# saiakarsh193/GenVox

Measured on AMD Instinct MI355X. Metric: mel-frames/sec (teacher-forced batch), higher is better.
Workload: dtype f32

## Files before the change

genvox_amd/csrc/gemm_f32.hip:

```cpp
#include "gvx_kernels.h"

#include <cstdlib>

namespace gvx {

using f32x16 = __attribute__((ext_vector_type(16))) float;

constexpr int BK32 = 32;

__device__ __forceinline__ long row_off(const RowMap& m, int row) {
    return (long)(row / m.R) * m.s1 + (long)(row % m.R) * m.s0;
}

template <int WR, int WC, int TM, int TN, bool KMAJ = false, int BK = BK32>
__device__ __forceinline__ void gemm_f32_body(const GemmParams& p, const int block_x, const int tid, float* smem) {
    constexpr int LDS_LD = BK + 4;
    static_assert(BK == 32 || (BK == 64 && !KMAJ), "k-tiles of 32, or 64 for the row-major form");
    constexpr int BM = WR * TM * 32;
    constexpr int BN = WC * TN * 32;
    constexpr int NT = WR * WC * 64;
    constexpr int TPR = BK / 4;
    constexpr int RPP = NT / TPR;
    constexpr int A_V4 = (BM + RPP - 1) / RPP;
    constexpr int B_V4 = (BN + RPP - 1) / RPP;
    static_assert(!KMAJ || NT == 256, "the K-major loaders are written for 256 threads");
    float* As = smem;
    float* Bs = smem + 2 * BM * LDS_LD;

    const int lane = tid & 63, wave = tid >> 6;
    const int wr = wave / WC, wc = wave % WC;
    const int r = lane & 31, h = lane >> 5;
    const int n_tiles = (p.N + BN - 1) / BN;
    const int mt = block_x / n_tiles, nt = block_x % n_tiles;
    const int m0 = p.m_begin + mt * BM, n0 = nt * BN;
    const int k_begin = p.splitk > 1 ? (int)blockIdx.y * p.kchunk : 0;
    const int k_end = p.splitk > 1 ? min(p.K, k_begin + p.kchunk) : p.K;
    const long slice = p.splitk > 1 ? 0 : (long)blockIdx.y;
    const float* const Ab = p.A + slice * p.a_slice;
    const float* const Wb = p.W + slice * p.w_slice;
    float* const Cout = p.C + (p.splitk > 1 ? (long)blockIdx.y * p.c_split : slice * p.c_slice);

    const int ld_row = tid / TPR, ld_c4 = tid % TPR;
    const float* a_ptr[A_V4]; bool a_ok[A_V4];
    const float* b_ptr[B_V4]; bool b_ok[B_V4];
    constexpr int A_MQ = BM / 4, B_NQ = BN / 4;
    constexpr int A_P = (8 * A_MQ + 255) / 256, B_P = (8 * B_NQ + 255) / 256;
    const int amq = tid % A_MQ, akq = tid / A_MQ, bnq = tid % B_NQ, bkq = tid / B_NQ;
    const int a_col = min(m0 + 4 * amq, p.M - 4), b_col = min(n0 + 4 * bnq, p.N - 4);
    int ak_g[A_P], ak_i[A_P], bk_g[B_P], bk_i[B_P];
    long a_safe = 0, b_safe = 0;
    float4 ka_reg[A_P][4], kb_reg[B_P][4];
    if (KMAJ) {
#pragma unroll
        for (int i = 0; i < A_P; ++i) { const int k = k_begin + 4 * (akq + (256 / A_MQ) * i); ak_g[i] = k / p.amap.R; ak_i[i] = k - ak_g[i] * p.amap.R; }
#pragma unroll
        for (int i = 0; i < B_P; ++i) { const int k = k_begin + 4 * (bkq + (256 / B_NQ) * i); bk_g[i] = k / p.wmap.R; bk_i[i] = k - bk_g[i] * p.wmap.R; }
        a_safe = row_off(p.amap, k_begin); b_safe = row_off(p.wmap, k_begin);
    }
    if (!KMAJ) {
#pragma unroll
        for (int i = 0; i < A_V4; ++i) {
            int m = m0 + ld_row + RPP * i;
            a_ok[i] = m < p.M;
            a_ptr[i] = Ab + (a_ok[i] ? row_off(p.amap, m) : 0);
        }
#pragma unroll
        for (int i = 0; i < B_V4; ++i) {
            int n = n0 + ld_row + RPP * i;
            b_ok[i] = n < p.N;
            b_ptr[i] = Wb + (b_ok[i] ? (long)n * p.ldw : 0);
        }
    }
    float4 a_reg[A_V4], b_reg[B_V4];

#define GEMM_KMAJ_LOAD(NP, QPP, KQ, KG, KI, MAP, SAFE, PTR, COL, REG)                                        \
        _Pragma("unroll") for (int i = 0; i < NP; ++i) {                                                    \
            const int c_ = KQ + QPP * i;                                                                    \
            if (c_ < BK / 4) {                                                                              \
                const int kq_ = (K0_) + 4 * c_;                                                             \
                int g_ = KG[i], x_ = KI[i];                                                                 \
                _Pragma("unroll") for (int j = 0; j < 4; ++j) {                                             \
                    const bool ok_ = kq_ + j < k_end;                                                       \
                    REG[i][j] = *reinterpret_cast<const float4*>(PTR + (ok_ ? (long)g_ * MAP.s1 + (long)x_ * MAP.s0 : SAFE) + COL); \
                    if (++x_ == MAP.R) { x_ = 0; ++g_; }                                                    \
                }                                                                                           \
                x_ = KI[i] + BK; g_ = KG[i];                                                                \
                while (x_ >= MAP.R) { x_ -= MAP.R; ++g_; }                                                  \
                KI[i] = x_; KG[i] = g_;                                                                     \
            }                                                                                               \
        }
#define GEMM_LOAD_TILE(K0)                                                                                  \
    if (KMAJ) {                                                                                             \
        const int K0_ = (K0);                                                                               \
        GEMM_KMAJ_LOAD(A_P, (256 / A_MQ), akq, ak_g, ak_i, p.amap, a_safe, Ab, a_col, ka_reg)              \
        GEMM_KMAJ_LOAD(B_P, (256 / B_NQ), bkq, bk_g, bk_i, p.wmap, b_safe, Wb, b_col, kb_reg)              \
    } else                                                                                                  \
    {                                                                                                       \
        const int k_ = (K0) + 4 * ld_c4;                                                                    \
        const bool k_ok_ = k_ < k_end;                                                                      \
        const long a_koff_ = (long)(k_ >> 3) * p.a_kblk + (k_ & 7);                                         \
        _Pragma("unroll") for (int i = 0; i < A_V4; ++i) {                                                  \
            if (BM % RPP != 0 && ld_row + RPP * i >= BM) continue;                                          \
            a_reg[i] = *reinterpret_cast<const float4*>(a_ptr[i] + (k_ok_ ? a_koff_ : 0));                  \
        }                                                                                                   \
        _Pragma("unroll") for (int i = 0; i < B_V4; ++i) {                                                  \
            if (BN % RPP != 0 && ld_row + RPP * i >= BN) continue;                                          \
            b_reg[i] = *reinterpret_cast<const float4*>(b_ptr[i] + (k_ok_ ? k_ : 0));                       \
        }                                                                                                   \
    }
#define GEMM_KMAJ_STORE(NP, QPP, KQ, SM, ROWS, RQ, REG, BUF)                                                 \
        _Pragma("unroll") for (int i = 0; i < NP; ++i) {                                                    \
            const int c_ = KQ + QPP * i;                                                                    \
            if (c_ < BK / 4) {                                                                              \
                float* d_ = &SM[((BUF) * ROWS + 4 * RQ) * LDS_LD + 4 * c_];                                 \
                const int kq_ = (KS_) + 4 * c_;    \
                const bool o0_ = kq_ < k_end, o1_ = kq_ + 1 < k_end, o2_ = kq_ + 2 < k_end, o3_ = kq_ + 3 < k_end;   \
                *reinterpret_cast<float4*>(d_) = make_float4(o0_ ? REG[i][0].x : 0.f, o1_ ? REG[i][1].x : 0.f, o2_ ? REG[i][2].x : 0.f, o3_ ? REG[i][3].x : 0.f);              \
                *reinterpret_cast<float4*>(d_ + LDS_LD) = make_float4(o0_ ? REG[i][0].y : 0.f, o1_ ? REG[i][1].y : 0.f, o2_ ? REG[i][2].y : 0.f, o3_ ? REG[i][3].y : 0.f);     \
                *reinterpret_cast<float4*>(d_ + 2 * LDS_LD) = make_float4(o0_ ? REG[i][0].z : 0.f, o1_ ? REG[i][1].z : 0.f, o2_ ? REG[i][2].z : 0.f, o3_ ? REG[i][3].z : 0.f); \
                *reinterpret_cast<float4*>(d_ + 3 * LDS_LD) = make_float4(o0_ ? REG[i][0].w : 0.f, o1_ ? REG[i][1].w : 0.f, o2_ ? REG[i][2].w : 0.f, o3_ ? REG[i][3].w : 0.f); \
            }                                                                                               \
        }
#define GEMM_STORE_TILE(BUF, K0)                                                                            \
    if (KMAJ) {                                                                                             \
        const int KS_ = (K0);                                                                               \
        GEMM_KMAJ_STORE(A_P, (256 / A_MQ), akq, As, BM, amq, ka_reg, BUF)                                   \
        GEMM_KMAJ_STORE(B_P, (256 / B_NQ), bkq, Bs, BN, bnq, kb_reg, BUF)                                   \
    } else                                                                                                  \
    {                                                                                                       \
        const bool s_ok_ = (K0) + 4 * ld_c4 < k_end;    \
        _Pragma("unroll") for (int i = 0; i < A_V4; ++i)                                                    \
            if (BM % RPP == 0 || ld_row + RPP * i < BM)                                                     \
                *reinterpret_cast<float4*>(&As[((BUF) * BM + ld_row + RPP * i) * LDS_LD + 4 * ld_c4]) =     \
                    make_float4(s_ok_ ? a_reg[i].x : 0.f, s_ok_ ? a_reg[i].y : 0.f, s_ok_ ? a_reg[i].z : 0.f, s_ok_ ? a_reg[i].w : 0.f); \
        _Pragma("unroll") for (int i = 0; i < B_V4; ++i)                                                    \
            if (BN % RPP == 0 || ld_row + RPP * i < BN)                                                     \
                *reinterpret_cast<float4*>(&Bs[((BUF) * BN + ld_row + RPP * i) * LDS_LD + 4 * ld_c4]) =     \
                    make_float4(s_ok_ ? b_reg[i].x : 0.f, s_ok_ ? b_reg[i].y : 0.f, s_ok_ ? b_reg[i].z : 0.f, s_ok_ ? b_reg[i].w : 0.f); \
    }
#define GEMM_COMPUTE_TILE(BUF) GEMM_COMPUTE_KGS(BUF, 0, BK / 8)
#define GEMM_COMPUTE_KGS(BUF, KG0, KG1)              \
    {                                                                                                       \
        const float* a_base = &As[((BUF) * BM + wr * TM * 32 + r) * LDS_LD + 4 * h];                        \
        const float* b_base = &Bs[((BUF) * BN + wc * TN * 32 + r) * LDS_LD + 4 * h];                        \
        _Pragma("unroll") for (int kg = (KG0); kg < (KG1); ++kg) {                                          \
            float4 af[TM], bf[TN];                                                                          \
            _Pragma("unroll") for (int i = 0; i < TM; ++i)                                                  \
                af[i] = *reinterpret_cast<const float4*>(a_base + i * 32 * LDS_LD + 8 * kg);                \
            _Pragma("unroll") for (int j = 0; j < TN; ++j)                                                  \
                bf[j] = *reinterpret_cast<const float4*>(b_base + j * 32 * LDS_LD + 8 * kg);                \
            _Pragma("unroll") for (int i = 0; i < TM; ++i)                                                  \
                _Pragma("unroll") for (int j = 0; j < TN; ++j) {                                            \
                    acc[i][j] = __builtin_amdgcn_mfma_f32_32x32x2f32(af[i].x, bf[j].x, acc[i][j], 0, 0, 0); \
                    acc[i][j] = __builtin_amdgcn_mfma_f32_32x32x2f32(af[i].y, bf[j].y, acc[i][j], 0, 0, 0); \
                    acc[i][j] = __builtin_amdgcn_mfma_f32_32x32x2f32(af[i].z, bf[j].z, acc[i][j], 0, 0, 0); \
                    acc[i][j] = __builtin_amdgcn_mfma_f32_32x32x2f32(af[i].w, bf[j].w, acc[i][j], 0, 0, 0); \
                }                                                                                           \
        }                                                                                                   \
    }

    f32x16 acc[TM][TN];
#pragma unroll
    for (int i = 0; i < TM; ++i)
#pragma unroll
        for (int j = 0; j < TN; ++j)
#pragma unroll
            for (int q = 0; q < 16; ++q) acc[i][j][q] = 0.f;

    const int nkt = (k_end - k_begin + BK - 1) / BK;
    GEMM_LOAD_TILE(k_begin)
    GEMM_STORE_TILE(0, k_begin)
    __syncthreads();
    int kt = 0;
    for (; kt + 1 < nkt; ++kt) {
        const int cur = kt & 1;
        GEMM_LOAD_TILE(k_begin + (kt + 1) * BK)
        __builtin_amdgcn_sched_barrier(0);
        GEMM_COMPUTE_KGS(cur, 0, BK / 8 - 1)
        __builtin_amdgcn_sched_barrier(0);
        GEMM_COMPUTE_KGS(cur, BK / 8 - 1, BK / 8)
        GEMM_STORE_TILE(cur ^ 1, k_begin + (kt + 1) * BK)
        __syncthreads();
    }
    GEMM_COMPUTE_TILE(kt & 1)
#undef GEMM_LOAD_TILE
#undef GEMM_KMAJ_LOAD
#undef GEMM_KMAJ_STORE
#undef GEMM_STORE_TILE
#undef GEMM_COMPUTE_TILE
#undef GEMM_COMPUTE_KGS

#pragma unroll
    for (int i = 0; i < TM; ++i) {
#pragma unroll
        for (int q = 0; q < 16; ++q) {
            const int m = m0 + (wr * TM + i) * 32 + (q & 3) + 8 * (q >> 2) + 4 * h;
            if (m >= p.M) continue;
            const long c_off = row_off(p.cmap, m);
            const int grp = m / p.cmap.R, idx = m - grp * p.cmap.R;
            const bool live = !p.row_len || idx < p.row_len[grp];
            const bool halo_front = p.c_halo > 0 && idx < p.c_halo;
            const bool halo_back = p.c_halo > 0 && idx >= p.cmap.R - p.c_halo;
            const long halo_step = (long)p.c_halo * p.cmap.s0;
#pragma unroll
            for (int j = 0; j < TN; ++j) {
                const int n = n0 + (wc * TN + j) * 32 + r;
                if (n >= p.N) continue;
                float v = acc[i][j][q];
                if (p.bias) v += p.bias[n];
                if (p.act == ACT_RELU) v = fmaxf(v, 0.f);
                else if (p.act == ACT_TANH) v = tanhf(v);
                if (p.keep) v = p.keep[(long)m * p.keep_ld + n] ? 2.f * v : 0.f;
                const long col = (long)(n >> 3) * p.c_nblk + (n & 7);
                Cout[c_off + col] = live ? v : 0.f;
                if (halo_front) Cout[c_off - halo_step + col] = 0.f;
                if (halo_back) Cout[c_off + halo_step + col] = 0.f;
            }
        }
    }
}

template <int WR, int WC, int TM, int TN, bool KMAJ = false, int BK = BK32>
__global__ __launch_bounds__(WR * WC * 64) void gemm_f32_kernel(GemmParams p) {
    extern __shared__ __attribute__((aligned(16))) float smem[];
    gemm_f32_body<WR, WC, TM, TN, KMAJ, BK>(p, (int)blockIdx.x, (int)threadIdx.x, smem);
}

template <int WR, int WC, int TM, int TN, int BK = BK32>
static size_t lds_bytes_cfg() { return (size_t)2 * (WR * TM * 32 + WC * TN * 32) * (BK + 4) * sizeof(float); }

template <int WR, int WC, int TM, int TN, bool KMAJ = false, int BK = BK32>
static hipError_t init_cfg() {
    return hipFuncSetAttribute(reinterpret_cast<const void*>(gemm_f32_kernel<WR, WC, TM, TN, KMAJ, BK>),
                               hipFuncAttributeMaxDynamicSharedMemorySize, (int)lds_bytes_cfg<WR, WC, TM, TN, BK>());
}

hipError_t gemm_init() {
    hipError_t e = init_cfg<2, 2, 2, 2>();
    if (e != hipSuccess) return e;
    e = init_cfg<2, 2, 1, 2>();
    if (e != hipSuccess) return e;
    e = init_cfg<4, 1, 1, 3>();
    if (e != hipSuccess) return e;
    e = init_cfg<2, 3, 1, 1>();
    if (e != hipSuccess) return e;
    e = init_cfg<4, 2, 1, 2>();
    if (e != hipSuccess) return e;
    e = init_cfg<2, 2, 1, 1>();
    if (e != hipSuccess) return e;
    e = init_cfg<2, 2, 2, 2, true>();
    if (e != hipSuccess) return e;
    e = init_cfg<2, 2, 1, 2, true>();
    if (e != hipSuccess) return e;
    return init_cfg<4, 1, 1, 1>();
}

template <int WR, int WC, int TM, int TN, bool KMAJ = false, int BK = BK32>
static hipError_t launch_cfg(const GemmParams& p, hipStream_t s) {
    constexpr int BM = WR * TM * 32, BN = WC * TN * 32;
    const int grid = ((p.M - p.m_begin + BM - 1) / BM) * ((p.N + BN - 1) / BN);
    gemm_f32_kernel<WR, WC, TM, TN, KMAJ, BK><<<dim3(grid, p.splitk > 1 ? p.splitk : p.slices > 1 ? p.slices : 1), dim3(WR * WC * 64), lds_bytes_cfg<WR, WC, TM, TN, BK>(), s>>>(p);
    return hipGetLastError();
}

static bool four_waves() {
    static const bool on = [] { const char* e = std::getenv("GVX_GEMM_8W"); return e && e[0] == '0'; }();
    return on;
}

GemmPlan plan_gemm(const GemmParams& p) {
    GemmPlan pl{hipSuccess, 0, 0};
    if (p.M <= 0 || p.N <= 0) return pl;
    if (p.slices > 1 && (p.splitk > 1 || p.kmajor || p.keep || p.slices > 65535)) { pl.err = hipErrorInvalidValue; return pl; }
    if (p.kmajor) {
        if ((p.M & 3) || (p.N & 3) || p.M < 4 || p.N < 4 || ((p.amap.s0 | p.amap.s1 | p.wmap.s0 | p.wmap.s1) & 3)) { pl.err = hipErrorInvalidValue; return pl; }
        const long t128 = (long)((p.M + 127) / 128) * ((p.N + 127) / 128);
        pl.tile = t128 < 384 ? 2212 : 2222;
        return pl;
    }
    if (p.K & 3) { pl.err = hipErrorInvalidValue; return pl; }
    if (p.N <= 32) { pl.tile = 4111; return pl; }
    if (p.N <= 96) {
        pl.tile = p.M - p.m_begin <= 4096 ? 2311 : 4113;
        return pl;
    }
    const long n_tiles = (long)((p.N + 127) / 128) * (p.slices > 1 ? p.slices : 1), tiles128 = (long)((p.M + 127) / 128) * n_tiles;
    if (tiles128 < 192) { pl.tile = 2211; return pl; }
    if (tiles128 < 384) { pl.tile = 2212; return pl; }
    pl.tile = four_waves() ? 2222 : 4212;
    const long rem = tiles128 % 256;
    if (p.splitk <= 1 && p.m_begin == 0 && rem > 0 && rem <= 64) {
        const long rows_big = ((tiles128 - rem) / n_tiles) * 128;
        if (rows_big > 0 && rows_big < p.M) pl.rows_big = (int)rows_big;
    }
    return pl;
}

static hipError_t launch_tile(int tile, const GemmParams& p, hipStream_t s) {
    switch (tile) {
        case 4111: return launch_cfg<4, 1, 1, 1>(p, s);
        case 2311: return launch_cfg<2, 3, 1, 1>(p, s);
        case 4113: return launch_cfg<4, 1, 1, 3>(p, s);
        case 2211: return launch_cfg<2, 2, 1, 1>(p, s);
        case 2212: return p.kmajor ? launch_cfg<2, 2, 1, 2, true>(p, s) : launch_cfg<2, 2, 1, 2>(p, s);
        case 2222: return p.kmajor ? launch_cfg<2, 2, 2, 2, true>(p, s) : launch_cfg<2, 2, 2, 2>(p, s);
        case 4212: return launch_cfg<4, 2, 1, 2>(p, s);
    }
    return hipErrorInvalidValue;
}

hipError_t launch_gemm(const GemmParams& p, hipStream_t s) {
    const GemmPlan pl = plan_gemm(p);
    if (pl.err != hipSuccess || pl.tile == 0) return pl.err;
    if (pl.rows_big == 0) return launch_tile(pl.tile, p, s);
    GemmParams a = p, b = p;
    a.M = pl.rows_big;
    b.m_begin = pl.rows_big;
    const hipError_t e = launch_tile(pl.tile, a, s);
    if (e != hipSuccess) return e;
    return launch_tile(2211, b, s);
}

void set_splitk(GemmParams& p, int splitk) {
    p.kchunk = ((p.K + splitk - 1) / splitk + 63) / 64 * 64;
    p.splitk = (p.K + p.kchunk - 1) / p.kchunk;
}

__global__ void splitk_reduce_kernel(const float* part, int splitk, long MN, int N, const float* bias, float* out, long ldc) {
    for (long i = (long)blockIdx.x * blockDim.x + threadIdx.x; i < MN; i += (long)gridDim.x * blockDim.x) {
        float v = part[i];
        for (int s = 1; s < splitk; ++s) v += part[(long)s * MN + i];
        const int n = (int)(i % N);
        if (bias) v += bias[n];
        out[(i / N) * ldc + n] = v;
    }
}

hipError_t launch_gemm_splitk(const GemmParams& p0, int splitk, float* scratch, hipStream_t s) {
    if (splitk <= 1) return launch_gemm(p0, s);
    if (p0.act != ACT_NONE || p0.keep || p0.row_len || p0.c_halo || p0.c_nblk != 8 || p0.cmap.s1 != 0 || p0.cmap.R < p0.M || !scratch)
        return hipErrorInvalidValue;
    GemmParams p = p0;
    set_splitk(p, splitk);
    p.C = scratch; p.cmap = RowMap{p.M, 0, (long)p.N};
    p.c_split = (long)p.M * p.N;
    p.bias = nullptr;
    hipError_t e = launch_gemm(p, s);
    if (e != hipSuccess) return e;
    const long MN = (long)p.M * p.N;
    long blocks = (MN + 255) / 256;
    if (blocks > 2048) blocks = 2048;
    splitk_reduce_kernel<<<dim3((unsigned)blocks), dim3(256), 0, s>>>(scratch, p.splitk, MN, p.N, p0.bias, p0.C, p0.cmap.s0);
    return hipGetLastError();
}

}
```

genvox_amd/csrc/gvx_api.hip:

```cpp
#include "gvx_internal.h"

namespace gvx {
#ifdef GVX_STAMPS
hipError_t read_stamps_skinny(unsigned long long* host96);
hipError_t read_stamps_attention(unsigned long long* host96);
hipError_t read_stamps_persist(unsigned long long* host96);
hipError_t read_wg_spans(unsigned long long* host1024);
hipError_t read_stamps_resident(unsigned long long* host480);
hipError_t read_wg_stamps_resident(unsigned long long* host896);
hipError_t read_wg_stamps_resident_ar(unsigned long long* host896);
hipError_t read_row_stamps_persist_ar(unsigned long long* host256);
hipError_t read_loc_stamps_persist(unsigned long long* host32);
hipError_t read_row_stamps_persist(unsigned long long* host512);
#endif
hipError_t skinny_init();
hipError_t gemm_init();
hipError_t attention_init();
hipError_t attention_persistent_init();
}

using namespace gvx;

namespace {
thread_local std::string g_err;
std::mutex g_capture_mutex;
}
namespace gvx {
int set_error(int code, const char* msg) { g_err = msg; return code; }

int fail(int code, const char* fmt, ...) {
    char buf[1024];
    va_list ap;
    va_start(ap, fmt);
    vsnprintf(buf, sizeof buf, fmt, ap);
    va_end(ap);
    g_err = buf;
    return code;
}

std::mutex& capture_mutex() { return g_capture_mutex; }

bool conv_uses_winograd(const gvx_model* m, int cin, int cout, int k) {
    if (m->winograd <= 0 || !winograd_shape_ok(cin, cout, k)) return false;
    return m->winograd >= 2 || cin >= WINOGRAD_MIN_CHANNELS;
}

size_t winograd_scratch_floats(const gvx_model* m, int B, int T) {
    bool any = false;
    for (int i = 0; i < m->d.postnet_n_conv; ++i) any = any || postnet_layer_winograd_shape(m->d, i);
    if (!any) return 0;
    const size_t tile = (size_t)2 * WINO_PTS * m->d.postnet_dim, all = (size_t)B * ((T + WINO_OUT - 1) / WINO_OUT) * tile;
    const size_t budget = WINOGRAD_GROUP_BYTES / sizeof(float) / tile * tile;
    return all <= budget ? all : budget > tile ? budget : tile;
}

WsPlan make_ws_plan(const gvx_model* m, int B, int L, int T, int mode) {
    const gvx_dims& d = m->d;
    const int E = d.embed_dim, H = E / 2, M = d.n_mels, P = d.prenet_dim, A = d.att_rnn_dim, D = d.dec_rnn_dim;
    const int pe = (d.enc_kernel - 1) / 2, pp = (d.postnet_kernel - 1) / 2;
    WsPlan w{};
    size_t off = 0;
    auto take = [&](size_t floats) { size_t o = off; off = align_up(off + floats * sizeof(float), 256); return o; };
    w.flags = take(128);
    w.sync = take(HANDOFF_WORDS);
    w.xa = take((size_t)B * (L + 2 * pe) * E);
    w.xb = take((size_t)B * (L + 2 * pe) * E);
    w.xg = take((size_t)B * L * 8 * H);
    w.enc_h = take((size_t)2 * 2 * B * H);
    w.enc_c = take((size_t)2 * B * H);
    w.memory = take((size_t)B * L * E);
    w.len_copy = take((size_t)B);
    w.pm = take((size_t)B * L * d.att_dim);
    w.frames = take((size_t)(T + 1) * B * M);
    w.pre1 = take((size_t)(T + 1) * B * P);
    w.prenet = take((size_t)(T + 1) * B * P);
    w.h_a = take((size_t)RS_HA_SLOTS * B * A);
    w.c_a = take((size_t)B * A);
    w.c_d = take((size_t)B * D);
    w.hc = take((size_t)(T + 1) * B * (D + E));
    w.w_cum = take((size_t)B * L);
    w.q_slab = take((size_t)(A / 8) * B * d.att_dim);
    w.proj = take((size_t)B * T * m->PSB());
    w.energies = take((size_t)B * L);
    w.align_tm = take((size_t)T * B * L);
    w.loc = take((size_t)B * L * d.att_dim);
    w.p_slab = take((size_t)(D / 8) * B * m->PSB());
    w.p_ctx = take((size_t)B * m->PSB());
    w.att_part = take((size_t)2 * B * 4 * A);
    w.dec_part = take((size_t)2 * B * 4 * D);
    w.pre_gate = take(mode == WS_TEACHER_FORCED && plan_teacher_forced(m, B, L, TF_INFERENCE).pre_gate ? (size_t)T * B * 4 * A : 0);
    w.xchg = take(attention_persistent_xchg_floats(B));
    w.ar_masks = take(((size_t)2 * T * B * P + 3) / 4);
    const int cmax = d.postnet_dim > M ? d.postnet_dim : M;
    w.ya = take((size_t)B * (T + 2 * pp) * cmax);
    w.yb = take((size_t)B * (T + 2 * pp) * cmax);
    w.total = off;
    return w;
}

gvx_model::GraphSet* touch_graph_set(gvx_model* m, std::vector<gvx_model::GraphSet>& cache, const gvx_model::LoopKey& key) {
    gvx_model::GraphSet* hit = nullptr;
    for (auto& gs : cache)
        if (gs.key == key) hit = &gs;
    if (!hit) {
        if (cache.size() >= gvx_model::GRAPH_SETS) {
            size_t lru = 0;
            for (size_t i = 1; i < cache.size(); ++i)
                if (cache[i].last_use < cache[lru].last_use) lru = i;
            for (auto e : cache[lru].execs)
                if (e) (void)hipGraphExecDestroy(e);
            cache.erase(cache.begin() + lru);
        }
        cache.emplace_back();
        hit = &cache.back();
        hit->key = key;
    }
    ++hit->sightings;
    hit->last_use = ++m->use_clock;
    return hit;
}

int check_common(const gvx_model* m, int B, int L, int T, void* ws, size_t ws_bytes, int mode) {
    if (!m) return fail(GVX_ERR_INVALID_ARG, "null model");
    if (!m->dev_blob) return fail(GVX_ERR_STATE, "weights not bound (call gvx_model_bind_blob)");
    if (B < 1 || B > 64) return fail(GVX_ERR_UNSUPPORTED, "batch %d not in [1, 64] (shard larger batches across calls / GPUs)", B);
    if (L < 1 || T < 1) return fail(GVX_ERR_INVALID_ARG, "L and T must be >= 1");
    if (!ws) return fail(GVX_ERR_WORKSPACE, "null workspace");
    if (reinterpret_cast<uintptr_t>(ws) & 255) return fail(GVX_ERR_WORKSPACE, "workspace must be 256-byte aligned");
    const size_t need = make_ws_plan(m, B, L, T, mode).total;
    if (ws_bytes < need) return fail(GVX_ERR_WORKSPACE, "workspace too small: %zu < %zu bytes", ws_bytes, need);
    if (!attention_supported(L, m->d.att_dim, m->d.att_loc_filters, m->d.att_loc_kernel, m->d.embed_dim))
        return fail(GVX_ERR_UNSUPPORTED, "L = %d is too long for the attention kernels' LDS budget", L);
    return GVX_OK;
}

}

namespace {

int check_dims(const gvx_dims& d) {
    if (d.n_tokens < 1) return fail(GVX_ERR_INVALID_ARG, "n_tokens must be >= 1");
    const int dims8[] = {d.embed_dim, d.prenet_dim, d.att_rnn_dim, d.dec_rnn_dim, d.att_dim, d.postnet_dim, d.n_mels};
    const char* names[] = {"embed_dim", "prenet_dim", "att_rnn_dim", "dec_rnn_dim", "att_dim", "postnet_dim", "n_mels"};
    for (int i = 0; i < 7; ++i)
        if (dims8[i] < 8 || dims8[i] % 8) return fail(GVX_ERR_UNSUPPORTED, "%s = %d must be a positive multiple of 8", names[i], dims8[i]);
    if (d.embed_dim % 16) return fail(GVX_ERR_UNSUPPORTED, "embed_dim = %d must be a multiple of 16 (BiLSTM halves are multiples of 8)", d.embed_dim);
    if (d.att_dim > 256) return fail(GVX_ERR_UNSUPPORTED, "att_dim = %d > 256 is not supported", d.att_dim);
    if (d.att_loc_filters < 1 || d.att_loc_filters > 32) return fail(GVX_ERR_UNSUPPORTED, "att_loc_filters = %d must be in [1, 32]", d.att_loc_filters);
    const int ks[] = {d.enc_kernel, d.att_loc_kernel, d.postnet_kernel};
    for (int k : ks)
        if (k < 1 || k % 2 == 0) return fail(GVX_ERR_UNSUPPORTED, "kernel size %d must be odd (the reference pads (k-1)/2 on both sides)", k);
    if (d.enc_n_conv < 1 || d.enc_n_conv > MAX_CONV || d.postnet_n_conv < 1 || d.postnet_n_conv > MAX_CONV)
        return fail(GVX_ERR_UNSUPPORTED, "number of convolutions must be in [1, %d]", MAX_CONV);
    return GVX_OK;
}

void read_knobs(gvx_model* m) {
    auto env = [](const char* name) { const char* e = std::getenv(name); return e ? e : ""; };
    auto flag = [&](const char* name, bool dflt) { const char c = env(name)[0]; return c == '\0' ? dflt : dflt ? c != '0' : c == '1'; };
    auto number = [&](const char* name, int dflt) { const char* e = env(name); return e[0] ? std::atoi(e) : dflt; };
    m->use_graph = !flag("GVX_NO_GRAPH", false);
    m->capture_first = flag("GVX_GRAPH_FIRST", false);
    m->attn_one_launch = !flag("GVX_ATTN_SPLIT", false);
    m->attn_persistent = flag("GVX_ATTN_PERSISTENT", true);
    for (const char* name : {"AMD_SERIALIZE_KERNEL", "HIP_LAUNCH_BLOCKING"})
        if (env(name)[0] != '\0' && env(name)[0] != '0') m->attn_persistent = false;
    m->ar_resident = flag("GVX_AR_RESIDENT", false);
    m->ar_split_h = flag("GVX_AR_SPLIT_H", true);
    m->enc_persistent = flag("GVX_ENC_PERSISTENT", true);
    m->enc_fork_after = number("GVX_ENC_FORK_AFTER", 1);
    m->train_resident = flag("GVX_TRAIN_RESIDENT", true);
    m->train_resident_loop = flag("GVX_TRAIN_RESIDENT_LOOP", true);
    m->tf_rows64 = flag("GVX_TF_ROWS64", false);
    m->tf_resident = flag("GVX_TF_RESIDENT", true);
    m->ar_resident_loop = flag("GVX_AR_RESIDENT_LOOP", true);
    m->tf_long_rows_224 = flag("GVX_TF_LONG_224", true);
    m->attn_prefetch = flag("GVX_ATTN_PREFETCH", true);
    m->pa_depth = number("GVX_PA_DEPTH", 4) == 6 ? 6 : 4;
    m->side_pool = env("GVX_SIDE_POOL")[0] == '2' ? 2u : 1u;
    m->spin_limit = (unsigned)std::strtoul(env("GVX_HANDOFF_SPIN_LIMIT"), nullptr, 10);
    m->rs_debug = number("GVX_RS_DEBUG", 0);
    m->debug_skip_resident = flag("GVX_DEBUG_SKIP_RESIDENT", false);
    m->debug_enc_skip_block = number("GVX_DEBUG_ENC_SKIP_BLOCK", -1);
    m->debug_plan = std::getenv("GVX_DEBUG_PLAN") != nullptr;
    m->winograd = number("GVX_CONV_WINOGRAD", 1);
    if (m->winograd < 0 || m->winograd > 2) m->winograd = 1;
}

}

extern "C" {

const char* gvx_last_error(void) { return g_err.c_str(); }
int gvx_version(void) { return 1; }

int gvx_model_create(const gvx_dims* dims, gvx_model** out) {
    if (!dims || !out) return fail(GVX_ERR_INVALID_ARG, "null argument");
    int rc = check_dims(*dims);
    if (rc != GVX_OK) return rc;
    gvx_model* m = new gvx_model();
    m->d = *dims;
    m->blob = make_blob_layout(*dims);
    read_knobs(m);
    *out = m;
    return GVX_OK;
}

void gvx_model_destroy(gvx_model* m) {
    if (m) {
        if (m->gather_off) (void)hipFree(m->gather_off);
        if (m->gather_tid) (void)hipFree(m->gather_tid);
    }
    if (!m) return;
    if (m->ev_valid)
        for (auto& e : m->ev) (void)hipEventDestroy(e);
    for (auto& e : m->kev) (void)hipEventDestroy(e);
    m->drop_graphs();
    if (m->cap_stream) (void)hipStreamDestroy(m->cap_stream);
    if (m->pa_fork) (void)hipEventDestroy(m->pa_fork);
    if (m->pa_join) (void)hipEventDestroy(m->pa_join);
    if (m->enc_mid) (void)hipEventDestroy(m->enc_mid);
    if (m->ar_done_host) (void)hipHostFree(m->ar_done_host);
    for (hipEvent_t e : m->ar_ev)
        if (e) (void)hipEventDestroy(e);
    delete m;
}

size_t gvx_model_blob_bytes(const gvx_model* m) { return m ? m->blob.total * sizeof(float) : 0; }

int gvx_model_bind_blob(gvx_model* m, const void* device_blob) {
    if (!m || !device_blob) return fail(GVX_ERR_INVALID_ARG, "null argument");
    if (reinterpret_cast<uintptr_t>(device_blob) & 255) return fail(GVX_ERR_INVALID_ARG, "blob must be 256-byte aligned");
    if (m->dev_blob != device_blob) m->drop_graphs();
    m->dev_blob = reinterpret_cast<const float*>(device_blob);
    HIP_TRY(gemm_init());
    HIP_TRY(skinny_init());
    HIP_TRY(attention_init());
    HIP_TRY(attention_persistent_init());
    HIP_TRY(decoder_resident_init());
    return GVX_OK;
}

size_t gvx_workspace_bytes(const gvx_model* m, int B, int L, int T) {
    if (!m || B < 1 || L < 1 || T < 1) return 0;
    return make_ws_plan(m, B, L, T).total;
}

size_t gvx_workspace_bytes_autoregressive(const gvx_model* m, int B, int L, int max_steps) {
    if (!m || B < 1 || L < 1 || max_steps < 1) return 0;
    return make_ws_plan(m, B, L, max_steps, WS_AUTOREGRESSIVE).total;
}

}

namespace {

int conv_layer(const gvx_model* m, const float* in, float* out, int B, int T, int cin, int cout, int k, size_t w_off, size_t b_off,
               int act, int out_halo, hipStream_t s) {
    const int p = (k - 1) / 2;
    GemmParams g{};
    g.A = in; g.amap = RowMap{T, (long)(T + 2 * p) * cin, (long)cin};
    g.W = m->dev_blob + w_off; g.ldw = (long)k * cin;
    g.C = out + (long)out_halo * cout; g.cmap = RowMap{T, (long)(T + 2 * out_halo) * cout, (long)cout};
    g.bias = m->dev_blob + b_off;
    g.M = B * T; g.N = cout; g.K = k * cin; g.act = act;
    HIP_TRY(launch_gemm(g, s));
    return GVX_OK;
}

int encoder_impl(gvx_model* m, const int64_t* tokens, const int32_t* lengths, int B, int L, float* memory_out, void* ws,
                 const WsPlan& wp, hipStream_t s, const float* conv_out = nullptr, float* c_seq_out = nullptr, float* xg_out = nullptr,
                 hipEvent_t dense_done = nullptr) {
    const gvx_dims& d = m->d;
    const int E = d.embed_dim, H = E / 2, pe = (d.enc_kernel - 1) / 2;
    float* xa = ws_ptr<float>(ws, wp.xa);
    float* xb = ws_ptr<float>(ws, wp.xb);
    float* xg = ws_ptr<float>(ws, wp.xg);
    float* enc_h = ws_ptr<float>(ws, wp.enc_h);
    float* enc_c = ws_ptr<float>(ws, wp.enc_c);
    int* flags = ws_ptr<int>(ws, wp.flags);
    float* cur = xa;
    float* nxt = xb;
    if (conv_out) {
        HIP_TRY(launch_to_channels_last(conv_out, xa, B, E, L, pe, nullptr, s));
    } else {
        HIP_TRY(launch_embed(tokens, m->dev_blob + m->blob.emb, d.n_tokens, xa, xb, B, L, E, pe, flags + FLAG_TOKEN, s));
        for (int i = 0; i < d.enc_n_conv; ++i) {
            if (dense_done && i == m->enc_fork_after) { HIP_TRY(hipEventRecord(dense_done, s)); dense_done = nullptr; }
            int rc = conv_layer(m, cur, nxt, B, L, E, E, d.enc_kernel, m->blob.enc_w[i], m->blob.enc_b[i], ACT_RELU, pe, s);
            if (rc != GVX_OK) return rc;
            float* t = cur; cur = nxt; nxt = t;
        }
    }
    if (dense_done) HIP_TRY(hipEventRecord(dense_done, s));
    {
        GemmParams g{};
        g.A = cur + (long)pe * E; g.amap = RowMap{L, (long)(L + 2 * pe) * E, (long)E};
        g.W = m->dev_blob + m->blob.enc_wih; g.ldw = E;
        g.C = xg; g.cmap = RowMap{B * L, 0, (long)8 * H};
        g.bias = m->dev_blob + m->blob.enc_bih;
        g.M = B * L; g.N = 8 * H; g.K = E; g.act = ACT_NONE;
        HIP_TRY(launch_gemm(g, s));
    }
    const bool resident = m->enc_persistent && encoder_persistent_supported(B, H);
    if (!resident) HIP_TRY(zero_async(enc_h, (size_t)4 * B * H * sizeof(float), s));
    if (!resident) HIP_TRY(zero_async(enc_c, (size_t)2 * B * H * sizeof(float), s));
    float* mem_ws = ws_ptr<float>(ws, wp.memory);
    if (!resident) HIP_TRY(zero_async(mem_ws, (size_t)B * L * E * sizeof(float), s));
    const int32_t* len_ws = nullptr;
    if (lengths) {
        int32_t* lc = ws_ptr<int32_t>(ws, wp.len_copy);
        HIP_TRY(hipMemcpyAsync(lc, lengths, (size_t)B * sizeof(int32_t), hipMemcpyDeviceToDevice, s));
        len_ws = lc;
    }
    auto enqueue = [&](hipStream_t st) -> int {
        for (int step = 0; step < L; ++step) {
            SkinnyJob jobs[2];
            for (int dir = 0; dir < 2; ++dir) {
                SkinnyJob& J = jobs[dir];
                std::memset(&J, 0, sizeof J);
                float* h_cur = enc_h + ((size_t)dir * 2 + (step & 1)) * B * H;
                float* h_nxt = enc_h + ((size_t)dir * 2 + ((step + 1) & 1)) * B * H;
                J.Wp = m->dev_blob + m->blob.enc_whh_frag[dir];
                J.x[0] = XSeg{h_cur, H};
                J.N = 4 * H; J.nkg = H / 8; J.mode = 0; J.B = B;
                J.c = enc_c + (size_t)dir * B * H;
                J.h_out = h_nxt;
                J.addend = xg + (size_t)dir * 4 * H; J.add_bs = (long)L * 8 * H; J.add_ts = 8 * H;
                J.lengths = len_ws; J.step = step; J.reverse = dir; J.seq_len = L;
                J.seq_out = mem_ws + (size_t)dir * H; J.seq_bs = (long)L * E; J.seq_ts = E;
                if (c_seq_out) J.c_seq_out = c_seq_out + (size_t)dir * H;
                J.h_prev = h_cur;
            }
            HIP_TRY(launch_skinny(jobs, 2, SK_ENCODER, st));
        }
        return GVX_OK;
    };
    if (resident) {
        unsigned* sync = ws_ptr<unsigned>(ws, wp.sync);
        void* const zp[2] = {enc_h, sync + HANDOFF_TIMEOUT};
        const size_t zb[2] = {(size_t)4 * B * H * sizeof(float), sizeof(unsigned)};
        HIP_TRY(launch_zero_many(zp, zb, 2, s));
        EncPersistParams ep{};
        ep.Wp[0] = m->dev_blob + m->blob.enc_whh_frag[0]; ep.Wp[1] = m->dev_blob + m->blob.enc_whh_frag[1];
        ep.xg = xg; ep.lengths = len_ws; ep.hx = enc_h; ep.seq_out = mem_ws; ep.c_seq_out = c_seq_out;
        ep.sync = sync; ep.spin_limit = m->spin_limit; ep.B = B; ep.L = L; ep.H = H;
        ep.debug_skip_block = m->debug_enc_skip_block;
        HIP_TRY(launch_encoder_persistent(ep, s));
        float* outs[2] = {mem_ws, c_seq_out};
        const size_t counts[2] = {(size_t)B * L * E, (size_t)B * L * E};
        HIP_TRY(launch_poison_on_timeout(sync + HANDOFF_TIMEOUT, flags + FLAG_TIMEOUT, outs, counts, c_seq_out ? 2 : 1, s));
    } else {
        const gvx_model::LoopKey key{ws, mem_ws, m->dev_blob, B, L, 0, lengths != nullptr};
        const int rc = run_chunk(m, m->use_graph && !c_seq_out ? touch_graph_set(m, m->enc_graphs, key) : nullptr, 0, s, enqueue);
        if (rc != GVX_OK) return rc;
    }
    if (xg_out) HIP_TRY(hipMemcpyAsync(xg_out, xg, (size_t)B * L * 8 * H * sizeof(float), hipMemcpyDeviceToDevice, s));
    if (memory_out != mem_ws)
        HIP_TRY(hipMemcpyAsync(memory_out, mem_ws, (size_t)B * L * E * sizeof(float), hipMemcpyDeviceToDevice, s));
    return GVX_OK;
}

int postnet_impl(gvx_model* m, const float* mel_in, const int32_t* mel_lengths, int B, int T, float* mel_post_out, float* ya,
                 float* yb, float* wino, size_t wino_floats, hipStream_t s) {
    const gvx_dims& d = m->d;
    const int M = d.n_mels, pp = (d.postnet_kernel - 1) / 2, n = d.postnet_n_conv;
    HIP_TRY(launch_to_channels_last(mel_in, ya, B, M, T, pp, mel_lengths, s));
    float* cur = ya;
    float* nxt = yb;
    for (int i = 0; i < n; ++i) {
        const int cin = i == 0 ? M : d.postnet_dim, cout = i == n - 1 ? M : d.postnet_dim;
        const bool last = i == n - 1;
        if (postnet_layer_winograd_shape(d, i) && conv_uses_winograd(m, cin, cout, d.postnet_kernel)) {
            const int C = cin;
            const long total = (long)B * ((T + WINO_OUT - 1) / WINO_OUT);
            const size_t tile = (size_t)2 * WINO_PTS * C, budget = WINOGRAD_GROUP_BYTES / sizeof(float);
            long fit = (long)((wino_floats < budget ? wino_floats : budget) / tile);
            if (fit < 1) return fail(GVX_ERR_WORKSPACE, "Postnet: %zu floats of scratch do not hold one Winograd tile (%zu)", wino_floats, tile);
            if (m->wino_group > 0 && m->wino_group < fit) fit = m->wino_group;
            if (fit > total) fit = total;
            const long groups = (total + fit - 1) / fit, per_group = (total + groups - 1) / groups;
            for (long mt0 = 0; mt0 < total; mt0 += per_group) {
                const long Mt = total - mt0 < per_group ? total - mt0 : per_group;
                float* V = wino;
                float* Mm = wino + (size_t)WINO_PTS * Mt * C;
                HIP_TRY(launch_winograd_input(cur, V, B, mt0, Mt, T, C, s));
                GemmParams g{};
                g.A = V; g.amap = RowMap{(int)Mt, 0, (long)C};
                g.W = m->dev_blob + m->blob.post_u[i]; g.ldw = C;
                g.C = Mm; g.cmap = RowMap{(int)Mt, 0, (long)C};
                g.bias = nullptr; g.M = (int)Mt; g.N = C; g.K = C; g.act = ACT_NONE;
                g.slices = WINO_PTS; g.a_slice = Mt * C; g.w_slice = (long)C * C; g.c_slice = Mt * C;
                HIP_TRY(launch_gemm(g, s));
                HIP_TRY(launch_winograd_output(Mm, m->dev_blob + m->blob.post_b[i], mel_lengths, nxt, B, mt0, Mt, T, C, s));
            }
            float* t = cur; cur = nxt; nxt = t;
            continue;
        }
        const int out_halo = last ? 0 : pp;
        const bool fused_halo = out_halo > 0 && T >= out_halo;
        if (out_halo > 0 && !fused_halo) HIP_TRY(launch_zero_halo(nxt, B, T, pp, cout, s));
        GemmParams g{};
        g.A = cur; g.amap = RowMap{T, (long)(T + 2 * pp) * cin, (long)cin};
        g.W = m->dev_blob + m->blob.post_w[i]; g.ldw = (long)d.postnet_kernel * cin;
        g.C = nxt + (long)out_halo * cout; g.cmap = RowMap{T, (long)(T + 2 * out_halo) * cout, (long)cout};
        g.bias = m->dev_blob + m->blob.post_b[i];
        g.M = B * T; g.N = cout; g.K = d.postnet_kernel * cin; g.act = last ? ACT_NONE : ACT_TANH;
        g.row_len = last ? nullptr : mel_lengths;
        g.c_halo = fused_halo ? out_halo : 0;
        HIP_TRY(launch_gemm(g, s));
        float* t = cur; cur = nxt; nxt = t;
    }
    HIP_TRY(launch_residual_to_channels_first(mel_in, cur, mel_post_out, B, M, T, mel_lengths, s));
    return GVX_OK;
}

struct PostnetPlan { size_t ya, yb, wino, wino_floats, total; };
PostnetPlan make_postnet_plan(const gvx_model* m, int B, int T) {
    const gvx_dims& d = m->d;
    const int pp = (d.postnet_kernel - 1) / 2, cmax = d.postnet_dim > d.n_mels ? d.postnet_dim : d.n_mels;
    const size_t buf = align_up((size_t)B * (T + 2 * pp) * cmax * sizeof(float), 256);
    PostnetPlan p;
    p.ya = align_up((128 + HANDOFF_WORDS) * sizeof(float), 256);
    p.yb = p.ya + buf;
    p.wino = p.yb + buf;
    const WsPlan w = make_ws_plan(m, B, 1, T, WS_AUTOREGRESSIVE);
    const size_t tile = (size_t)2 * WINO_PTS * d.postnet_dim, room = (w.ya - w.xa) / sizeof(float) / tile * tile;
    p.wino_floats = winograd_scratch_floats(m, B, T);
    if (p.wino_floats > room) p.wino_floats = room > tile ? room : tile;
    p.total = p.wino + align_up(p.wino_floats * sizeof(float), 256);
    return p;
}

}

extern "C" {

int gvx_teacher_forced_rows_per_call(const gvx_model* m, int L) {
    if (!m) return 0;
    return plan_teacher_forced(m, 64, L, TF_INFERENCE).kind != 0 ? 64 : 32;
}

int gvx_teacher_forced_resident(const gvx_model* m, int B, int L) {
    if (!m || B < 1 || L < 1) return 0;
    return plan_teacher_forced(m, B, L, TF_INFERENCE).kind != 0 ? 1 : 0;
}

int gvx_teacher_forced_loop_kind(const gvx_model* m, int B, int L) {
    if (!m || B < 1 || L < 1) return 0;
    return plan_teacher_forced(m, B, L, TF_INFERENCE).kind;
}

int gvx_autoregressive_loop_kind(const gvx_model* m, int B, int L) {
    if (!m || B < 1 || L < 1) return 0;
    return plan_autoregressive(m, B, L).kind;
}

int gvx_autoregressive_windowed_loop_kind(const gvx_model* m, int B, int L) {
    if (!m || B < 1 || L < 1) return 0;
    return plan_autoregressive(m, B, L, true).kind;
}

int gvx_debug_decoder_plan_windowed(const gvx_model* m, int B, int L, int* out) {
    if (!m || !out) return fail(GVX_ERR_INVALID_ARG, "null argument");
    if (B < 1 || L < 1) return fail(GVX_ERR_INVALID_ARG, "B, L >= 1 (got %d, %d)", B, L);
    const ArLoopPlan a = plan_autoregressive(m, B, L, true);
    out[0] = a.kind; out[1] = a.split_h; out[2] = a.fold; out[3] = a.graph;
    return GVX_OK;
}

int gvx_debug_decoder_plan(const gvx_model* m, int mode, int B, int L, int* out) {
    if (!m || !out) return fail(GVX_ERR_INVALID_ARG, "null argument");
    if (mode < 0 || mode > 2 || B < 1 || L < 1) return fail(GVX_ERR_INVALID_ARG, "mode must be 0, 1 or 2 and B, L >= 1 (got %d, %d, %d)", mode, B, L);
    const TfLoopPlan t = plan_teacher_forced(m, B, L, (TfMode)mode);
    const ArLoopPlan a = plan_autoregressive(m, B, L);
    const int v[12] = {t.kind, t.pa_layout, t.tile_layout, t.rows64, t.pre_gate, t.timeout_check, t.side_stream, t.graph,
                       a.kind, a.split_h, a.fold, a.graph};
    for (int i = 0; i < 12; ++i) out[i] = v[i];
    return GVX_OK;
}

long long gvx_debug_graph_replays(const gvx_model* m) { return m ? (long long)m->graph_replays : -1; }

int gvx_debug_encoder_resident(const gvx_model* m, int B) {
    if (!m || B < 1) return 0;
    return m->enc_persistent && encoder_persistent_supported(B, m->H()) ? 1 : 0;
}

int gvx_model_set_persistent_attention(gvx_model* m, int enable) {
    if (!m) return fail(GVX_ERR_INVALID_ARG, "null argument");
    m->attn_persistent = enable != 0;
    return GVX_OK;
}

int gvx_model_set_winograd(gvx_model* m, int mode) {
    if (!m) return fail(GVX_ERR_INVALID_ARG, "null argument");
    if (mode < 0 || mode > 2) return fail(GVX_ERR_INVALID_ARG, "winograd mode must be 0, 1 or 2 (got %d)", mode);
    m->winograd = mode;
    return GVX_OK;
}

int gvx_debug_conv_plan(const gvx_model* m, int cin, int cout, int k) {
    if (!m || cin < 1 || cout < 1 || k < 1) return -1;
    return conv_uses_winograd(m, cin, cout, k) ? 1 : 0;
}

int gvx_debug_set_winograd_group(gvx_model* m, int tiles) {
    if (!m || tiles < 0) return fail(GVX_ERR_INVALID_ARG, "bad argument");
    m->wino_group = tiles;
    return GVX_OK;
}

int gvx_debug_winograd_constants(double* at, double* g, double* bt) {
    if (!at || !g || !bt) return fail(GVX_ERR_INVALID_ARG, "null argument");
    for (int i = 0; i < WINO_OUT; ++i)
        for (int s = 0; s < WINO_PTS; ++s) at[i * WINO_PTS + s] = wino_AT(i, s);
    for (int s = 0; s < WINO_PTS; ++s) {
        for (int k = 0; k < WINO_TAPS; ++k) g[s * WINO_TAPS + k] = wino_G(s, k);
        for (int i = 0; i < WINO_PTS; ++i) bt[s * WINO_PTS + i] = wino_BT(s, i);
    }
    return GVX_OK;
}

int gvx_model_set_resident_kernels(gvx_model* m, int enable) {
    if (!m) return fail(GVX_ERR_INVALID_ARG, "null argument");
    m->attn_persistent = m->enc_persistent = m->tf_resident = enable != 0;
    if (!enable) m->ar_resident = false;
    return GVX_OK;
}

int gvx_workspace_status(const gvx_model* m, void* ws, size_t ws_bytes, void* stream, int32_t* host_out) {
    if (!m || !ws || !host_out) return fail(GVX_ERR_INVALID_ARG, "null argument");
    const WsPlan wp = make_ws_plan(m, 1, 1, 1, WS_AUTOREGRESSIVE);
    if (ws_bytes < wp.flags + 4 * sizeof(int32_t)) return fail(GVX_ERR_WORKSPACE, "workspace too small");
    hipStream_t s = (hipStream_t)stream;
    int32_t h[4] = {0, 0, 0, 0}, tmo = 0;
    int32_t* flags = ws_ptr<int32_t>(ws, wp.flags);
    HIP_TRY(hipMemcpyAsync(h, flags, sizeof h, hipMemcpyDeviceToHost, s));
    if (ws_bytes >= wp.sync + HANDOFF_WORDS * sizeof(unsigned))
        HIP_TRY(hipMemcpyAsync(&tmo, reinterpret_cast<const char*>(ws) + wp.sync + HANDOFF_TIMEOUT * sizeof(unsigned), sizeof tmo,
                               hipMemcpyDeviceToHost, s));
    HIP_TRY(zero_async(flags + FLAG_TOKEN, sizeof(int32_t), s));
    HIP_TRY(zero_async(flags + FLAG_TIMEOUT, sizeof(int32_t), s));
    if (ws_bytes >= wp.sync + HANDOFF_WORDS * sizeof(unsigned))
        HIP_TRY(zero_async(ws_ptr<unsigned>(ws, wp.sync) + HANDOFF_TIMEOUT, sizeof(unsigned), s));
    HIP_TRY(hipStreamSynchronize(s));
    host_out[0] = h[FLAG_TOKEN];
    host_out[1] = h[FLAG_TIMEOUT] ? h[FLAG_TIMEOUT] : tmo;
    return GVX_OK;
}

int gvx_encoder_forward(gvx_model* m, const int64_t* tokens, const int32_t* lengths, int B, int L, float* memory_out,
                        void* ws, size_t ws_bytes, void* stream) {
    int rc = check_common(m, B, L, 1, ws, ws_bytes, WS_AUTOREGRESSIVE);
    if (rc != GVX_OK) return rc;
    if (!tokens || !memory_out) return fail(GVX_ERR_INVALID_ARG, "null argument");
    return encoder_impl(m, tokens, lengths, B, L, memory_out, ws, make_ws_plan(m, B, L, 1, WS_AUTOREGRESSIVE), (hipStream_t)stream);
}

int gvx_decoder_teacher_forced(gvx_model* m, const float* memory, const int32_t* lengths, int B, int L, const float* mel_in, int T,
                               const uint8_t* keep_masks, float* mel_out, float* gate_out, float* align_out, void* ws,
                               size_t ws_bytes, void* stream) {
    int rc = check_common(m, B, L, T, ws, ws_bytes);
    if (rc != GVX_OK) return rc;
    if (!memory || !mel_in || !keep_masks || !mel_out || !gate_out || !align_out) return fail(GVX_ERR_INVALID_ARG, "null argument");
    const WsPlan wp = make_ws_plan(m, B, L, T);
    rc = decoder_tf_impl(m, memory, lengths, B, L, mel_in, T, keep_masks, mel_out, gate_out, align_out, ws, wp, (hipStream_t)stream);
    if (rc != GVX_OK) return rc;
    float* outs[3] = {mel_out, gate_out, align_out};
    const size_t counts[3] = {(size_t)B * m->d.n_mels * T, (size_t)B * T, (size_t)B * T * L};
    return poison_if_timed_out(m, B, L, ws, wp, outs, counts, 3, (hipStream_t)stream);
}

int gvx_encoder_lstm_forward(gvx_model* m, const float* conv_out, const int32_t* lengths, int B, int L, float* memory_out,
                             float* cell_states_out, float* input_preact_out, void* ws, size_t ws_bytes, void* stream) {
    int rc = check_common(m, B, L, 1, ws, ws_bytes, WS_AUTOREGRESSIVE);
    if (rc != GVX_OK) return rc;
    if (!conv_out || !memory_out) return fail(GVX_ERR_INVALID_ARG, "null argument");
    if (cell_states_out) HIP_TRY(zero_async(cell_states_out, (size_t)B * L * m->d.embed_dim * sizeof(float), (hipStream_t)stream));
    return encoder_impl(m, nullptr, lengths, B, L, memory_out, ws, make_ws_plan(m, B, L, 1, WS_AUTOREGRESSIVE), (hipStream_t)stream, conv_out,
                        cell_states_out, input_preact_out);
}

int gvx_decoder_teacher_forced_train(gvx_model* m, const float* memory, const int32_t* lengths, int B, int L, const float* mel_in, int T,
                                     const uint8_t* keep_masks, const uint8_t* att_keep, const uint8_t* dec_keep, float p_att, float p_dec,
                                     float* mel_out, float* gate_out, float* align_out, float* att_hidden_all, float* att_cell_all,
                                     float* dec_cell_all, float* dec_hidden_context_all, float* att_preact_all, float* dec_preact_all,
                                     void* ws, size_t ws_bytes, void* stream) {
    int rc = check_common(m, B, L, T, ws, ws_bytes);
    if (rc != GVX_OK) return rc;
    if (!memory || !mel_in || !keep_masks || !att_keep || !dec_keep || !mel_out || !gate_out || !align_out) return fail(GVX_ERR_INVALID_ARG, "null argument");
    if (!(p_att >= 0.f && p_att < 1.f && p_dec >= 0.f && p_dec < 1.f)) return fail(GVX_ERR_INVALID_ARG, "dropout probabilities must be in [0, 1)");
    if (plan_teacher_forced(m, B, L, TF_TRAIN_PARTIAL_TAPE).rows64)
        return fail(GVX_ERR_UNSUPPORTED, "training mode with %d rows on a GVX_TF_ROWS64 handle: the 64-row loop has no dropout and no tape (at most 32 rows per call)", B);
    hipStream_t s = (hipStream_t)stream;
    const int A = m->d.att_rnn_dim, D = m->d.dec_rnn_dim, E = m->d.embed_dim;
    const LstmDropout tr{att_keep, dec_keep, 1.f / (1.f - p_att), 1.f / (1.f - p_dec), att_hidden_all, att_cell_all, dec_cell_all, att_preact_all, dec_preact_all};
    if (att_hidden_all) HIP_TRY(zero_async(att_hidden_all, (size_t)B * A * sizeof(float), s));
    if (att_cell_all) HIP_TRY(zero_async(att_cell_all, (size_t)B * A * sizeof(float), s));
    if (dec_cell_all) HIP_TRY(zero_async(dec_cell_all, (size_t)B * D * sizeof(float), s));
    const WsPlan wp = make_ws_plan(m, B, L, T);
    rc = decoder_tf_impl(m, memory, lengths, B, L, mel_in, T, keep_masks, mel_out, gate_out, align_out, ws, wp, s, false, &tr);
    if (rc != GVX_OK) return rc;
    {
        float* outs[3] = {mel_out, gate_out, align_out};
        const size_t counts[3] = {(size_t)B * m->d.n_mels * T, (size_t)B * T, (size_t)B * T * L};
        rc = poison_if_timed_out(m, B, L, ws, wp, outs, counts, 3, s);
        if (rc != GVX_OK) return rc;
    }
    if (dec_hidden_context_all)
        HIP_TRY(hipMemcpyAsync(dec_hidden_context_all, ws_ptr<float>(ws, wp.hc), (size_t)(T + 1) * B * (D + E) * sizeof(float),
                               hipMemcpyDeviceToDevice, s));
    return GVX_OK;
}

int gvx_train_export(const gvx_model* m, const void* ws_c, size_t ws_bytes, int B, int L, int T, int what, float* dst, void* stream) {
    void* ws = const_cast<void*>(ws_c);
    if (!m || !ws || !dst) return fail(GVX_ERR_INVALID_ARG, "null argument");
    const WsPlan wp = make_ws_plan(m, B, L, T);
    if (ws_bytes < wp.total) return fail(GVX_ERR_WORKSPACE, "workspace too small");
    const gvx_dims& d = m->d;
    hipStream_t s = (hipStream_t)stream;
    const size_t rows = (size_t)(T + 1) * B;
    switch (what) {
        case 0: HIP_TRY(hipMemcpyAsync(dst, ws_ptr<float>(ws, wp.frames), rows * d.n_mels * sizeof(float), hipMemcpyDeviceToDevice, s)); break;
        case 1: HIP_TRY(hipMemcpyAsync(dst, ws_ptr<float>(ws, wp.pre1), rows * d.prenet_dim * sizeof(float), hipMemcpyDeviceToDevice, s)); break;
        case 2: return gvx_train_unblock(ws_ptr<float>(ws, wp.prenet), dst, T + 1, B, d.prenet_dim, stream);
        case 3: HIP_TRY(hipMemcpyAsync(dst, ws_ptr<float>(ws, wp.pm), (size_t)B * L * d.att_dim * sizeof(float), hipMemcpyDeviceToDevice, s)); break;
        default: return fail(GVX_ERR_INVALID_ARG, "gvx_train_export: unknown buffer %d", what);
    }
    return GVX_OK;
}

size_t gvx_postnet_workspace_bytes(const gvx_model* m, int B, int T) {
    if (!m || B < 1 || T < 1) return 0;
    return make_postnet_plan(m, B, T).total;
}

int gvx_postnet_forward(gvx_model* m, const float* mel_in, const int32_t* mel_lengths, int B, int T, float* mel_post_out, void* ws,
                        size_t ws_bytes, void* stream) {
    if (!m) return fail(GVX_ERR_INVALID_ARG, "null model");
    if (!m->dev_blob) return fail(GVX_ERR_STATE, "weights not bound (call gvx_model_bind_blob)");
    if (B < 1 || T < 1) return fail(GVX_ERR_INVALID_ARG, "B and T must be >= 1");
    if ((long)B * T > (1L << 30)) return fail(GVX_ERR_UNSUPPORTED, "B * T = %ld frames exceed the GEMM row index range", (long)B * T);
    if (!ws) return fail(GVX_ERR_WORKSPACE, "null workspace");
    if (reinterpret_cast<uintptr_t>(ws) & 255) return fail(GVX_ERR_WORKSPACE, "workspace must be 256-byte aligned");
    const PostnetPlan pp = make_postnet_plan(m, B, T);
    if (ws_bytes < pp.total) return fail(GVX_ERR_WORKSPACE, "workspace too small: %zu < %zu bytes", ws_bytes, pp.total);
    if (!mel_in || !mel_post_out) return fail(GVX_ERR_INVALID_ARG, "null argument");
    return postnet_impl(m, mel_in, mel_lengths, B, T, mel_post_out, ws_ptr<float>(ws, pp.ya), ws_ptr<float>(ws, pp.yb), ws_ptr<float>(ws, pp.wino), pp.wino_floats,
                        (hipStream_t)stream);
}

int gvx_mask_padding(float* mel, float* mel_post, float* gate, const int32_t* mel_lengths, int B, int n_mels, int T, void* stream) {
    if (!mel_lengths || B < 1 || T < 1 || n_mels < 1) return fail(GVX_ERR_INVALID_ARG, "bad argument");
    HIP_TRY(launch_mask_padding(mel, mel_post, gate, mel_lengths, B, n_mels, T, (hipStream_t)stream));
    return GVX_OK;
}

int gvx_tacotron2_forward(gvx_model* m, const int64_t* tokens, const int32_t* token_lengths, int B, int L, const float* mel_in,
                          const int32_t* mel_lengths, int T, const uint8_t* keep_masks, float* mel_out, float* mel_post_out,
                          float* gate_out, float* align_out, void* ws, size_t ws_bytes, void* stream) {
    int rc = check_common(m, B, L, T, ws, ws_bytes);
    if (rc != GVX_OK) return rc;
    if (!tokens || !mel_in || !keep_masks || !mel_out || !gate_out || !align_out)
        return fail(GVX_ERR_INVALID_ARG, "null argument");
    hipStream_t s = (hipStream_t)stream;
    const WsPlan wp = make_ws_plan(m, B, L, T);
    const bool timed = m->timing && m->ev_valid;
    float* memory = ws_ptr<float>(ws, wp.memory);
    if (timed) HIP_TRY(hipEventRecord(m->ev[0], s));
    const bool overlap = plan_teacher_forced(m, B, L, TF_INFERENCE).side_stream;
    if (overlap) {
        rc = ensure_side_stream(m);
        if (rc != GVX_OK) return rc;
        HIP_TRY(hipEventRecord(m->pa_fork, s));
        HIP_TRY(hipStreamWaitEvent(m->pa_stream, m->pa_fork, 0));
        rc = encoder_impl(m, tokens, token_lengths, B, L, memory, ws, wp, m->pa_stream, nullptr, nullptr, nullptr, m->enc_mid);
        if (rc != GVX_OK) return rc;
        rc = decoder_init_states(m, memory, B, L, decoder_buffers(ws, wp), m->pa_stream);
        if (rc != GVX_OK) return rc;
        HIP_TRY(hipEventRecord(m->pa_join, m->pa_stream));
        HIP_TRY(hipStreamWaitEvent(s, m->enc_mid, 0));
        rc = decoder_prenet_part(m, B, L, mel_in, T, keep_masks, ws, wp, s);
        if (rc != GVX_OK) return rc;
        HIP_TRY(hipStreamWaitEvent(s, m->pa_join, 0));
    } else {
        rc = encoder_impl(m, tokens, token_lengths, B, L, memory, ws, wp, s);
        if (rc != GVX_OK) return rc;
    }
    if (timed) HIP_TRY(hipEventRecord(m->ev[1], s));
    rc = decoder_tf_impl(m, memory, token_lengths, B, L, mel_in, T, keep_masks, mel_out, gate_out, align_out, ws, wp, s, overlap);
    if (rc != GVX_OK) return rc;
    if (timed) HIP_TRY(hipEventRecord(m->ev[4], s));
    if (mel_post_out) {
        rc = postnet_impl(m, mel_out, nullptr, B, T, mel_post_out, ws_ptr<float>(ws, wp.ya), ws_ptr<float>(ws, wp.yb), ws_ptr<float>(ws, wp.xa),
                          (wp.ya - wp.xa) / sizeof(float), s);
        if (rc != GVX_OK) return rc;
        if (mel_lengths) HIP_TRY(launch_mask_padding(mel_out, mel_post_out, gate_out, mel_lengths, B, m->d.n_mels, T, s));
    }
    float* outs[4] = {mel_out, gate_out, align_out, mel_post_out};
    const size_t nm = (size_t)B * m->d.n_mels * T;
    const size_t counts[4] = {nm, (size_t)B * T, (size_t)B * T * L, nm};
    rc = poison_if_timed_out(m, B, L, ws, wp, outs, counts, mel_post_out ? 4 : 3, s);
    if (rc != GVX_OK) return rc;
    if (timed) HIP_TRY(hipEventRecord(m->ev[5], s));
    return GVX_OK;
}

int gvx_tacotron2_loss(const float* mel_out, const float* mel_post_out, const float* gate_out, const float* mel_target,
                       const float* gate_target, int B, int n_mels, int T, float* loss_out, void* scratch, size_t scratch_bytes,
                       void* stream) {
    if (!mel_out || !mel_post_out || !gate_out || !mel_target || !gate_target || !loss_out || !scratch)
        return fail(GVX_ERR_INVALID_ARG, "null argument");
    if (B < 1 || n_mels < 1 || T < 1) return fail(GVX_ERR_INVALID_ARG, "B, n_mels and T must be >= 1");
    if (scratch_bytes < loss_scratch_bytes() || (reinterpret_cast<uintptr_t>(scratch) & 7))
        return fail(GVX_ERR_WORKSPACE, "scratch too small (%zu bytes needed) or not 8-byte aligned", loss_scratch_bytes());
    HIP_TRY(launch_tacotron2_loss(mel_out, mel_post_out, gate_out, mel_target, gate_target, (long)B * n_mels * T, (long)B * T,
                                  reinterpret_cast<double*>(scratch), loss_out, (hipStream_t)stream));
    return GVX_OK;
}

int gvx_prenet_masks_generate(uint8_t* masks_out, size_t n, uint64_t seed, void* stream) {
    if (!masks_out) return fail(GVX_ERR_INVALID_ARG, "null argument");
    HIP_TRY(launch_mask_gen(masks_out, n, seed, (hipStream_t)stream));
    return GVX_OK;
}

int gvx_stage_timing_enable(gvx_model* m, int enable) {
    if (!m) return fail(GVX_ERR_INVALID_ARG, "null model");
    if (enable && !m->ev_valid) {
        for (auto& e : m->ev) HIP_TRY(hipEventCreate(&e));
        m->ev_valid = true;
    }
    m->timing = enable != 0;
    return GVX_OK;
}

int gvx_kernel_timing_enable(gvx_model* m, int enable) {
    if (!m) return fail(GVX_ERR_INVALID_ARG, "null model");
    m->ktiming = enable != 0;
    return GVX_OK;
}

int gvx_kernel_times_ms(gvx_model* m, float* lstm_avg_ms, float* attn_avg_ms, int* n_steps) {
    if (!m || !lstm_avg_ms || !attn_avg_ms) return fail(GVX_ERR_INVALID_ARG, "null argument");
    if (m->n_lstm_ev < 1) return fail(GVX_ERR_STATE, "no timed decoder loop has run");
    HIP_TRY(hipEventSynchronize(m->kev[2]));
    float a = 0, b = 0;
    HIP_TRY(hipEventElapsedTime(&a, m->kev[0], m->kev[1]));
    HIP_TRY(hipEventElapsedTime(&b, m->kev[1], m->kev[2]));
    *lstm_avg_ms = a / m->n_lstm_ev;
    *attn_avg_ms = m->n_attn_ev > 0 ? b / m->n_attn_ev : 0.f;
    if (n_steps) *n_steps = m->n_lstm_ev;
    return GVX_OK;
}

int gvx_stage_times_ms(gvx_model* m, float* t5, int* launches) {
    if (!m || !t5) return fail(GVX_ERR_INVALID_ARG, "null argument");
    if (!m->ev_valid) return fail(GVX_ERR_STATE, "stage timing was not enabled");
    HIP_TRY(hipEventSynchronize(m->ev[5]));
    for (int i = 0; i < 5; ++i) HIP_TRY(hipEventElapsedTime(&t5[i], m->ev[i], m->ev[i + 1]));
    if (launches) *launches = m->last_decoder_launches;
    return GVX_OK;
}
#ifdef GVX_STAMPS
int gvx_debug_read_stamps_skinny(unsigned long long* host96) {
    HIP_TRY(hipDeviceSynchronize());
    HIP_TRY(gvx::read_stamps_skinny(host96));
    return GVX_OK;
}
int gvx_debug_read_stamps_persist(unsigned long long* host96) {
    HIP_TRY(hipDeviceSynchronize());
    HIP_TRY(gvx::read_stamps_persist(host96));
    return GVX_OK;
}
int gvx_debug_read_wg_spans(unsigned long long* host1024) {
    HIP_TRY(hipDeviceSynchronize());
    HIP_TRY(gvx::read_wg_spans(host1024));
    return GVX_OK;
}
int gvx_debug_read_stamps_resident(unsigned long long* host480) {
    HIP_TRY(hipDeviceSynchronize());
    HIP_TRY(gvx::read_stamps_resident(host480));
    return GVX_OK;
}
int gvx_debug_read_wg_stamps_resident(unsigned long long* host896, unsigned long long* rows512) {
    HIP_TRY(hipDeviceSynchronize());
    HIP_TRY(gvx::read_wg_stamps_resident(host896));
    HIP_TRY(gvx::read_row_stamps_persist(rows512));
    return GVX_OK;
}
int gvx_debug_read_loc_stamps(unsigned long long* host32) {
    HIP_TRY(hipDeviceSynchronize());
    HIP_TRY(gvx::read_loc_stamps_persist(host32));
    return GVX_OK;
}
int gvx_debug_read_stamps_ar(unsigned long long* host896, unsigned long long* rows256) {
    HIP_TRY(hipDeviceSynchronize());
    HIP_TRY(gvx::read_wg_stamps_resident_ar(host896));
    HIP_TRY(gvx::read_row_stamps_persist_ar(rows256));
    return GVX_OK;
}
int gvx_debug_read_stamps(unsigned long long* host96) {
    HIP_TRY(hipDeviceSynchronize());
    unsigned long long tmp[96];
    HIP_TRY(gvx::read_stamps_skinny(host96));
    HIP_TRY(gvx::read_stamps_attention(tmp));
    for (int i = 32; i < 96; ++i) host96[i] = tmp[i];
    return GVX_OK;
}
#endif

}
```

genvox_amd/csrc/gvx_internal.h:

```cpp
#pragma once
#include "../../include/genvox_amd.h"
#include "gvx_kernels.h"
#include "winograd_f45.h"

#include <cmath>
#include <cstdarg>
#include <cstdio>
#include <cstdlib>
#include <cstring>
#include <mutex>
#include <string>
#include <unordered_map>
#include <vector>

namespace gvx {

int fail(int code, const char* fmt, ...);

#define HIP_TRY(expr)                                                                          \
    do {                                                                                       \
        hipError_t _e = (expr);                                                                \
        if (_e != hipSuccess) return fail(GVX_ERR_HIP, "%s failed: %s", #expr, hipGetErrorString(_e)); \
    } while (0)

constexpr int MAX_CONV = 8;
constexpr double BN_EPS = 1e-5;

struct Blob {
    size_t emb;
    size_t enc_w[MAX_CONV], enc_b[MAX_CONV];
    size_t enc_wih, enc_bih, enc_whh_frag[2];
    size_t pre_w0, pre_w1, pre_w0_t, pre_w1_t;
    size_t att_frag, att_bias, att_wpre, wq_t, wmem, v, loc_conv, loc_dense;
    size_t dec_frag, dec_bias;
    size_t proj_w, proj_b, proj_frag, proj_hd_t, proj_ctx_frag, proj_ctx_t;
    size_t post_w[MAX_CONV], post_b[MAX_CONV];
    size_t post_u[MAX_CONV];
    size_t total;
};
inline bool winograd_shape_ok(int cin, int cout, int k) { return k == WINO_TAPS && cin == cout && cin % 32 == 0; }
inline bool postnet_layer_winograd_shape(const gvx_dims& d, int i) {
    return i > 0 && i < d.postnet_n_conv - 1 && winograd_shape_ok(d.postnet_dim, d.postnet_dim, d.postnet_kernel);
}
Blob make_blob_layout(const gvx_dims& d);

inline size_t frag_floats(int N, int K) { return (size_t)((N + 31) / 32) * (K / 8) * 64 * 4; }

struct WsPlan {
    size_t xa, xb, xg, enc_h, enc_c, flags, sync, memory;
    size_t pm, frames, pre1, prenet, h_a, c_a, c_d, hc, w_cum, q_slab, proj, energies, align_tm, len_copy, loc, ar_masks, p_slab, p_ctx;
    size_t att_part, dec_part, pre_gate, xchg;
    size_t ya, yb;
    size_t total;
};

}

struct gvx_model {
    gvx_dims d;
    gvx::Blob blob;
    const float* dev_blob = nullptr;
    bool use_graph = true;
    bool capture_first = false;
    bool attn_one_launch = true;
    bool attn_persistent = true;
    bool ar_resident = false;
    bool enc_persistent = true;
    bool ar_split_h = true;
    bool tf_rows64 = false;
    bool tf_resident = true;
    bool ar_resident_loop = true;
    bool tf_long_rows_224 = true;
    bool train_resident = true;
    bool train_resident_loop = true;
    bool attn_prefetch = true;
    int winograd = 1;
    int wino_group = 0;
    int enc_fork_after = 1;
    int pa_depth = 4;
    unsigned side_pool = 1;
    unsigned spin_limit = 0;
    int rs_debug = 0;
    bool debug_skip_resident = false;
    int debug_enc_skip_block = -1;
    bool debug_plan = false;
    bool timing = false;
    hipEvent_t ev[6] = {nullptr, nullptr, nullptr, nullptr, nullptr, nullptr};
    bool ev_valid = false;
    int last_decoder_launches = 0;
    struct LoopKey {
        const void* ws; const void* memory; const void* blob; int B, L, T; bool has_len;
        float threshold = 0.f;
        int variant = 0;
        const void* centres = nullptr; int win_back = 0, win_ahead = 0;
        bool operator==(const LoopKey& o) const {
            return ws == o.ws && memory == o.memory && blob == o.blob && B == o.B && L == o.L && T == o.T &&
                   has_len == o.has_len && threshold == o.threshold && variant == o.variant && centres == o.centres &&
                   win_back == o.win_back && win_ahead == o.win_ahead;
        }
    };
    struct GraphSet {
        LoopKey key;
        int sightings = 0;
        uint64_t last_use = 0;
        std::vector<hipGraphExec_t> execs;
    };
    static constexpr size_t GRAPH_SETS = 4;
    std::vector<GraphSet> ar_graphs, loop_graphs, enc_graphs;
    uint64_t use_clock = 0;
    uint64_t graph_replays = 0;
    hipStream_t pa_stream = nullptr;
    hipEvent_t pa_fork = nullptr, pa_join = nullptr, enc_mid = nullptr;
    int32_t* ar_done_host = nullptr;
    hipEvent_t ar_ev[2] = {nullptr, nullptr};
    std::vector<std::string> gather_names;
    std::vector<int64_t> gather_numel;
    int32_t* gather_off = nullptr;
    uint8_t* gather_tid = nullptr;
    void drop_graphs() {
        for (auto* c : {&ar_graphs, &loop_graphs, &enc_graphs}) {
            for (auto& gs : *c)
                for (auto e : gs.execs)
                    if (e) (void)hipGraphExecDestroy(e);
            c->clear();
        }
    }
    hipStream_t cap_stream = nullptr;
    bool ktiming = false;
    std::vector<hipEvent_t> kev;
    int n_lstm_ev = 0, n_attn_ev = 0;
    int reserve_events(size_t n) {
        while (kev.size() < n) {
            hipEvent_t e;
            if (hipEventCreate(&e) != hipSuccess) return GVX_ERR_HIP;
            kev.push_back(e);
        }
        return GVX_OK;
    }
    int H() const { return d.embed_dim / 2; }
    int PS() const { return (d.n_mels + 1 + 3) & ~3; }
    int PSB() const { return (d.n_mels + 1 + 7) & ~7; }
};

namespace gvx {

enum TfMode : int { TF_INFERENCE = 0, TF_TRAIN_WHOLE_TAPE = 1, TF_TRAIN_PARTIAL_TAPE = 2 };
struct TfLoopPlan {
    int kind;
    int pa_layout;
    int tile_layout;
    bool rows64;
    bool pre_gate;
    bool timeout_check;
    bool side_stream;
    bool graph;
};
struct ArLoopPlan {
    int kind;
    bool split_h;
    bool fold;
    bool graph;
};
TfLoopPlan plan_teacher_forced(const gvx_model* m, int B, int L, TfMode mode);
ArLoopPlan plan_autoregressive(const gvx_model* m, int B, int L, bool windowed = false);

enum WsMode : int { WS_TEACHER_FORCED = 0, WS_AUTOREGRESSIVE = 1 };

constexpr int WINOGRAD_MIN_CHANNELS = 256;
constexpr size_t WINOGRAD_GROUP_BYTES = (size_t)128 << 20;
bool conv_uses_winograd(const gvx_model* m, int cin, int cout, int k);
size_t winograd_scratch_floats(const gvx_model* m, int B, int T);

constexpr int FLAG_TOKEN = 0;
constexpr int FLAG_AR_DONE = 1;
constexpr int FLAG_TIMEOUT = 2;
constexpr int FLAG_AR_FRAMES = 64;

WsPlan make_ws_plan(const gvx_model* m, int B, int L, int T, int mode = WS_TEACHER_FORCED);
int check_common(const gvx_model* m, int B, int L, int T, void* ws, size_t ws_bytes, int mode = WS_TEACHER_FORCED);

template <typename T>
T* ws_ptr(void* ws, size_t off) { return reinterpret_cast<T*>(reinterpret_cast<char*>(ws) + off); }

inline hipError_t zero_async(void* p, size_t bytes, hipStream_t s) { return hipMemsetAsync(p, 0, bytes, s); }

gvx_model::GraphSet* touch_graph_set(gvx_model* m, std::vector<gvx_model::GraphSet>& cache, const gvx_model::LoopKey& key);
std::mutex& capture_mutex();

template <class F>
int run_chunk(gvx_model* m, gvx_model::GraphSet* gs, size_t chunk, hipStream_t s, F&& enqueue) {
    if (!m->use_graph || !gs || (gs->sightings < 2 && !m->capture_first)) return enqueue(s);
    if (gs->execs.size() <= chunk) gs->execs.resize(chunk + 1, nullptr);
    hipGraphExec_t exec = gs->execs[chunk];
    if (!exec) {
        std::lock_guard<std::mutex> lock(capture_mutex());
        hipGraph_t graph = nullptr;
        if (!m->cap_stream) HIP_TRY(hipStreamCreateWithFlags(&m->cap_stream, hipStreamNonBlocking));
        HIP_TRY(hipStreamBeginCapture(m->cap_stream, hipStreamCaptureModeThreadLocal));
        const int rc = enqueue(m->cap_stream);
        const hipError_t ce = hipStreamEndCapture(m->cap_stream, &graph);
        if (rc != GVX_OK) { if (graph) (void)hipGraphDestroy(graph); return rc; }
        HIP_TRY(ce);
        HIP_TRY(hipGraphInstantiate(&exec, graph, nullptr, nullptr, 0));
        HIP_TRY(hipGraphDestroy(graph));
        gs->execs[chunk] = exec;
    }
    HIP_TRY(hipGraphLaunch(exec, s));
    ++m->graph_replays;
    return GVX_OK;
}

struct DecoderBuffers {
    float *pm, *frames, *pre1, *prenet, *h_a, *c_a, *c_d, *hc, *w_cum, *q_slab, *proj, *energies, *align_tm, *loc, *p_slab, *p_ctx;
    float *att_part, *dec_part, *pre_gate;
    int32_t* len_copy;
};
DecoderBuffers decoder_buffers(void* ws, const WsPlan& wp);

struct LstmDropout {
    const uint8_t* att_keep; const uint8_t* dec_keep; float att_scale, dec_scale;
    float* h_a_all; float* c_a_all; float* c_d_all;
    float* pre_a_all; float* pre_d_all;
};

int ensure_side_stream(gvx_model* m);
int decoder_init_states(gvx_model* m, const float* memory, int B, int L, const DecoderBuffers& db, hipStream_t s);
int decoder_prenet_part(gvx_model* m, int B, int L, const float* mel_in, int T, const uint8_t* keep_masks, void* ws, const WsPlan& wp,
                        hipStream_t s);
int decoder_tf_impl(gvx_model* m, const float* memory, const int32_t* lengths, int B, int L, const float* mel_in, int T,
                    const uint8_t* keep_masks, float* mel_out, float* gate_out, float* align_out, void* ws, const WsPlan& wp,
                    hipStream_t s, bool prenet_done = false, const LstmDropout* train = nullptr);
int poison_if_timed_out(const gvx_model* m, int B, int L, void* ws, const WsPlan& wp, float* const* outs, const size_t* counts, int n,
                        hipStream_t s);

}
```

genvox_amd/csrc/gvx_kernels.h:

```cpp
#pragma once
#include <hip/hip_runtime.h>
#include <stddef.h>
#include <stdint.h>

#ifdef GVX_STAMPS
namespace gvx { namespace { __device__ unsigned long long gvx_stamps[3][32]; } }
#define GVX_STAMP(k, i)                                                                         \
    do {                                                                                        \
        if (blockIdx.x == 0 && blockIdx.y == 0 && threadIdx.x == 0) gvx::gvx_stamps[k][i] = wall_clock64(); \
    } while (0)
#else
#define GVX_STAMP(k, i) do { } while (0)
#endif

namespace gvx {

int set_error(int code, const char* msg);

inline size_t align_up(size_t x, size_t a) { return (x + a - 1) / a * a; }

enum Act : int { ACT_NONE = 0, ACT_RELU = 1, ACT_TANH = 2 };

struct RowMap {
    int R;
    long s1, s0;
};

struct GemmParams {
    const float* A; RowMap amap; long a_kblk = 8;
    const float* W; long ldw;
    float* C; RowMap cmap; long c_nblk = 8;
    const float* bias;
    const uint8_t* keep; long keep_ld;
    int M, N, K;
    int act;
    int splitk = 1; int kchunk = 0; long c_split = 0;
    bool kmajor = false; RowMap wmap{1, 0, 0};
    int m_begin = 0;
    const int32_t* row_len = nullptr;
    int c_halo = 0;
    int slices = 1; long a_slice = 0, w_slice = 0, c_slice = 0;
};
hipError_t launch_gemm(const GemmParams& p, hipStream_t s);
struct GemmPlan { hipError_t err; int tile; int rows_big; };
GemmPlan plan_gemm(const GemmParams& p);
void set_splitk(GemmParams& p, int splitk);
hipError_t launch_gemm_splitk(const GemmParams& p, int splitk, float* scratch, hipStream_t s);

struct XSeg { const float* p; int len; };

struct SkinnyJob {
    const float* Wp;
    const float* bias;
    XSeg x[3];
    int N;
    int nkg;
    int kg0, nkg_w;
    int mode;
    float* c;
    float* h_out;
    const float* addend; long add_bs, add_ts;
    const float* addend2;
    const int32_t* lengths; int step; int reverse; int seq_len;
    float* seq_out; long seq_bs, seq_ts;
    const float* h_prev;
    const uint8_t* h_keep; float h_scale;
    float* c_out; float* c_seq_out;
    float* pre_out;
    const float* Wq_t;
    float* q_slab; int att_dim;
    const float* xw; const float* xsrc;
    int defer_seg;
    const unsigned* ctx_cnt; unsigned ctx_target;
    unsigned* start_cnt;
    const unsigned* ready_cnt; unsigned ready_target;
    unsigned* tmo;
    unsigned spin_limit;
    float* y;
    const uint8_t* keep; long keep_stride;
    int act;
    int B;
};
struct LocJob {
    const float* w_prev; long w_prev_bs;
    const float* w_cum;
    const float* loc_conv_t;
    const float* loc_dense_t;
    const float* pm;
    float* loc_out;
    int B, L, a, kl, G;
};
enum SkinnyKind : int { SK_DECODER = 0, SK_ENCODER = 1, SK_AR = 2, SK_TRAIN = 3 };
hipError_t launch_skinny(const SkinnyJob* jobs, int njobs, int kind, hipStream_t s, const LocJob* loc = nullptr);
struct AttnParams;
hipError_t launch_skinny_attn(const SkinnyJob* jobs, int njobs, const AttnParams& ap, hipStream_t s);
struct EncPersistParams {
    const float* Wp[2];
    const float* xg;
    const int32_t* lengths;
    float* hx;
    float* seq_out;
    float* c_seq_out;
    unsigned* sync;
    unsigned spin_limit;
    int B, L, H;
    int debug_skip_block;
};
bool encoder_persistent_supported(int B, int H);
hipError_t launch_encoder_persistent(const EncPersistParams& p, hipStream_t s);
hipError_t launch_skinny_pa(const SkinnyJob& att, const SkinnyJob* dec, hipStream_t s, int depth = 4, int layout = 1);
hipError_t launch_skinny_pa64(const SkinnyJob* jobs, int njobs, hipStream_t s);

struct AttnParams {
    const float* q_slab; int n_slabs;
    float* w_cum;
    const float* loc;
    const float* v;
    const float* pm;
    const float* memory;
    const int32_t* lengths;
    float* energies;
    float* w_out; long w_out_bs;
    float* ctx_out;
    int B, L, a, F, kl, E, G;
    const float* pf_w[2]; int pf_nkg[2]; int pf_tiles0, pf_tiles;
    const int32_t* c_prev; int32_t* c_out; long c_bs; int win_back, win_ahead;
};
hipError_t launch_attention(const AttnParams& p, hipStream_t s);
hipError_t launch_attention_step(const AttnParams& p, hipStream_t s);
int attention_slices(int B, int E);
int attention_groups(int B, int L);
bool attention_supported(int L, int a, int F, int kl, int E);

constexpr int HANDOFF_CNT_Q = 0, HANDOFF_CNT_CTX = 1024, HANDOFF_READY = 2048, HANDOFF_TIMEOUT = 3072;
constexpr int HANDOFF_STOP = 3072 + 512;
constexpr int HANDOFF_PAIR = 4096;
constexpr int HANDOFF_WORDS = 69632;
constexpr unsigned HANDOFF_SPIN_LIMIT = 200000u;
struct AttnPersistParams {
    const float* q_slab; int n_slabs;
    const float* v; const float* pm; const float* memory; const int32_t* lengths;
    const float* loc_conv_t; const float* loc_dense_t;
    float* w_out; long w_out_bs, w_out_ts;
    float* ctx_base; long ctx_ts;
    unsigned* sync;
    int B, L, T, kl;
    unsigned spin_limit;
    float* xchg;
    unsigned q_first;
    const unsigned* q_flags; int n_q_flags;
    unsigned* ctx_flags;
    int debug;
    const float* p_slab; int PSB, n_mels;
    const float* proj_b;
    float* proj_out;
    const float* pre_w0_t;
    const uint8_t* keep0;
    float* y1;
    int32_t* n_frames; int32_t* n_done; float gate_threshold;
    const unsigned* p_flags;
    unsigned* y1_flags;
    int32_t* centres; int win_back, win_ahead;
};
constexpr int RS_REP = 32;
constexpr int RS_FLAG_ATT = 8192;
constexpr int RS_FLAG_DEC = RS_FLAG_ATT + RS_REP * 128;
constexpr int RS_REP1 = 8;
constexpr int RS_FLAG_CTX = RS_FLAG_DEC + RS_REP * 128;
constexpr int RS_FLAG_Q = RS_FLAG_CTX + RS_REP1 * 32 * 32;
constexpr int RS_FLAG_Y1 = RS_FLAG_Q + RS_REP1 * 96 * 32;
constexpr int RS_REP_PRE = 8;
constexpr int RS_FLAG_PRE = RS_FLAG_Y1 + 32 * 32;
constexpr int RS_REP_P = 4;
constexpr int RS_FLAG_P = RS_FLAG_PRE + RS_REP_PRE * 8 * 32;
static_assert(RS_FLAG_P + RS_REP_P * 128 * 32 <= HANDOFF_WORDS, "flag replicas inside the hand-off block");
constexpr int RS_HA_SLOTS = 8;
struct DecResidentParams {
    const float* att_frag; const float* att_bias; const float* wq_t;
    const float* dec_frag; const float* dec_bias;
    const float* pre_gate;
    float* h_a;
    float* hc;
    float* q_slab;
    float* c_a; float* c_d;
    unsigned* sync;
    unsigned att_frag_bytes, dec_frag_bytes;
    int B, T;
    unsigned spin_limit;
    int debug;
    int kg_pre;
    int layout;
    const uint8_t* tr_keep_a; const uint8_t* tr_keep_d; float tr_scale_a, tr_scale_d;
    float* tr_c_a; float* tr_c_d; float* tr_pre_a; float* tr_pre_d;
};
struct ArResidentParams {
    const float* att_frag; const float* att_bias; const float* wq_t;
    const float* dec_frag; const float* dec_bias;
    const float* proj_hd_t;
    const float* proj_ctx_t;
    const float* pre_w1;
    const uint8_t* keep1;
    float* prenet;
    const float* y1;
    float* h_a; float* hc; float* q_slab;
    float* p_slab;
    float* c_a; float* c_d;
    const int32_t* n_done;
    unsigned* sync;
    unsigned att_frag_bytes;
    int B, T, PSB;
    unsigned spin_limit;
    int debug;
};
bool decoder_resident_supported(int B, int L);
hipError_t launch_decoder_ar_resident(const ArResidentParams& p, hipStream_t s);
hipError_t decoder_resident_init();
hipError_t launch_decoder_resident(const DecResidentParams& p, hipStream_t s);

bool attention_persistent_supported(int B, int L, int a, int F, int kl, int E, int att_rnn_dim, int dec_rnn_dim);
int attention_persistent_layout(int B, int L);
int attention_persistent_slabs(int layout);
int attention_persistent_workgroups(int B, int L);
size_t attention_persistent_xchg_floats(int B);
hipError_t attention_persistent_init();
hipError_t launch_attention_persistent(const AttnPersistParams& p, hipStream_t s);
hipError_t launch_handoff_set(unsigned* word, hipStream_t s);

#if defined(__HIPCC__)
typedef __attribute__((ext_vector_type(4))) unsigned gvx_u32x4;
__device__ __forceinline__ __amdgpu_buffer_rsrc_t make_rsrc(const void* p) {
    return __builtin_amdgcn_make_buffer_rsrc(const_cast<void*>(p), 0, 0x7fffffff, 0x00020000);
}
__device__ __forceinline__ float4 load_sc1(__amdgpu_buffer_rsrc_t r, unsigned byte_off) {
    const gvx_u32x4 v = __builtin_amdgcn_raw_buffer_load_b128(r, (int)byte_off, 0, 16);
    return make_float4(__uint_as_float(v.x), __uint_as_float(v.y), __uint_as_float(v.z), __uint_as_float(v.w));
}
__device__ __forceinline__ float load_sc1_f32(__amdgpu_buffer_rsrc_t r, unsigned byte_off) {
    return __uint_as_float(__builtin_amdgcn_raw_buffer_load_b32(r, (int)byte_off, 0, 16));
}
__device__ __forceinline__ void store_sc1(__amdgpu_buffer_rsrc_t r, unsigned byte_off, float4 v) {
    gvx_u32x4 u;
    u.x = __float_as_uint(v.x); u.y = __float_as_uint(v.y); u.z = __float_as_uint(v.z); u.w = __float_as_uint(v.w);
    __builtin_amdgcn_raw_buffer_store_b128(u, r, (int)byte_off, 0, 16);
}
template <bool FEW_WAITERS = false>
__device__ __forceinline__ bool handoff_wait(const unsigned* cnt, unsigned target, unsigned* tmo, unsigned code, unsigned limit = 0u,
                                             const unsigned* stop = nullptr) {
    if (limit == 0u) limit = HANDOFF_SPIN_LIMIT;
    unsigned spins = 0;
    while (__hip_atomic_load(cnt, __ATOMIC_RELAXED, __HIP_MEMORY_SCOPE_AGENT) < target) {
        ++spins;
        if ((spins & (FEW_WAITERS ? 127u : 7u)) == 1u) {
            if (__hip_atomic_load(tmo, __ATOMIC_RELAXED, __HIP_MEMORY_SCOPE_AGENT) != 0u) return false;
            if (stop && __hip_atomic_load(stop, __ATOMIC_RELAXED, __HIP_MEMORY_SCOPE_AGENT) != 0u) return false;
            if (spins > (FEW_WAITERS ? 16u : 1u) * limit) {
                __hip_atomic_store(tmo, code, __ATOMIC_RELAXED, __HIP_MEMORY_SCOPE_AGENT);
                return false;
            }
        }
        if (FEW_WAITERS || spins < 8u) __builtin_amdgcn_s_sleep(FEW_WAITERS ? 2 : 8);
        else __builtin_amdgcn_s_sleep(64);
    }
    return true;
}
#endif

hipError_t launch_embed(const int64_t* tokens, const float* emb, int n_tokens, float* x, float* x2, int B, int L, int E, int halo,
                        int* err_flag, hipStream_t s);
hipError_t launch_frames_from_mel(const float* mel_in, float* frames, int B, int M, int T, hipStream_t s);
hipError_t launch_split_projection(const float* proj, float* mel_out, float* gate_out, int B, int M, int T, hipStream_t s);
hipError_t launch_to_channels_last(const float* src, float* dst, int B, int M, int T, int halo, const int32_t* lens, hipStream_t s);
hipError_t launch_residual_to_channels_first(const float* mel, const float* y, float* mel_post, int B, int M, int T,
                                             const int32_t* lens, hipStream_t s);
hipError_t launch_zero_halo(float* buf, int B, int T, int halo, int C, hipStream_t s);
hipError_t launch_winograd_input(const float* x, float* V, int B, long mt0, long nmt, int T, int C, hipStream_t s);
hipError_t launch_winograd_output(const float* M, const float* bias, const int32_t* row_len, float* y, int B, long mt0, long nmt, int T, int C, hipStream_t s);
hipError_t launch_mask_padding(float* mel, float* mel_post, float* gate, const int32_t* mel_lengths, int B, int M, int T,
                               hipStream_t s);
hipError_t launch_zero_many(void* const* ptrs, const size_t* bytes, int n_arrays, hipStream_t s);
hipError_t launch_poison_on_timeout(const unsigned* tmo, int* sticky, float* const* ptrs, const size_t* counts, int n_arrays, hipStream_t s);
hipError_t launch_permute01(const float* src, float* dst, int T, int B, int n, hipStream_t s);
size_t loss_scratch_bytes();
hipError_t launch_tacotron2_loss(const float* mel, const float* mel_post, const float* gate, const float* mel_t, const float* gate_t,
                                 long n_mel, long n_gate, double* scratch, float* out3, hipStream_t s);
hipError_t launch_mask_gen(uint8_t* out, size_t n, uint64_t seed, hipStream_t s);
hipError_t launch_ar_stop(const float* proj_t, int gate_col, float threshold, int t, int B,
                          int32_t* n_frames, int32_t* n_done, hipStream_t s);
hipError_t launch_ar_project(const float* p_slab, int n_slabs, const float* p_ctx, float* proj_t, int M, float threshold, int t, int B,
                             int32_t* n_frames, int32_t* n_done, const float* w0t, const float* w1t, int P, const uint8_t* keep0,
                             const uint8_t* keep1, float* prenet_out, hipStream_t s);
hipError_t launch_ar_centres_finish(int32_t* centres, const int32_t* n_frames, const unsigned* tmo, int B, int T, hipStream_t s);
hipError_t launch_ar_emit_all(const float* proj, float* mel_out, float* gate_out, int B, int M, int Tmax, int steps,
                              const int32_t* n_frames, hipStream_t s);
hipError_t launch_permute01_partial(const float* src, float* dst, int steps, int Tdst, int B, int n, const int32_t* n_frames,
                                    hipStream_t s);

}
```

genvox_amd/csrc/gvx_pack.hip:

```cpp
#include "gvx_internal.h"

using namespace gvx;

namespace gvx {

Blob make_blob_layout(const gvx_dims& d) {
    Blob b{};
    size_t off = 0;
    auto take = [&](size_t n) { size_t o = off; off = align_up(off + n, 64); return o; };
    const int E = d.embed_dim, H = E / 2, M = d.n_mels, P = d.prenet_dim, A = d.att_rnn_dim, D = d.dec_rnn_dim;
    b.emb = take((size_t)d.n_tokens * E);
    for (int i = 0; i < d.enc_n_conv; ++i) { b.enc_w[i] = take((size_t)E * d.enc_kernel * E); b.enc_b[i] = take(E); }
    b.enc_wih = take((size_t)8 * H * E);
    b.enc_bih = take((size_t)8 * H);
    for (int dir = 0; dir < 2; ++dir) b.enc_whh_frag[dir] = take(frag_floats(4 * H, H));
    b.pre_w0 = take((size_t)P * M); b.pre_w1 = take((size_t)P * P);
    b.pre_w0_t = take((size_t)M * P);
    b.pre_w1_t = take((size_t)P * P);
    b.att_frag = take(frag_floats(4 * A, P + E + A)); b.att_bias = take((size_t)4 * A);
    b.att_wpre = take((size_t)4 * A * P);
    b.wq_t = take((size_t)A * d.att_dim);
    b.wmem = take((size_t)d.att_dim * E); b.v = take(d.att_dim);
    b.loc_conv = take((size_t)2 * d.att_loc_kernel * 32);
    b.loc_dense = take((size_t)32 * d.att_dim);
    b.dec_frag = take(frag_floats(4 * D, A + E + D)); b.dec_bias = take((size_t)4 * D);
    b.proj_w = take((size_t)(M + 1) * (D + E)); b.proj_b = take(M + 1);
    b.proj_frag = take(frag_floats(M + 1, D + E));
    b.proj_hd_t = take((size_t)D * ((M + 1 + 7) & ~7));
    b.proj_ctx_frag = take(frag_floats(M + 1, E));
    b.proj_ctx_t = take((size_t)(E / 4) * ((M + 1 + 7) & ~7) * 4);
    for (int i = 0; i < d.postnet_n_conv; ++i) {
        const int cin = i == 0 ? M : d.postnet_dim, cout = i == d.postnet_n_conv - 1 ? M : d.postnet_dim;
        b.post_w[i] = take((size_t)cout * d.postnet_kernel * cin);
        b.post_b[i] = take(cout);
    }
    for (int i = 0; i < d.postnet_n_conv; ++i)
        if (postnet_layer_winograd_shape(d, i)) b.post_u[i] = take((size_t)WINO_PTS * d.postnet_dim * d.postnet_dim);
    b.total = off;
    return b;
}

}

namespace {

void pack_frag(const std::vector<float>& W, int N, int K, float* out) {
    const int ntiles = (N + 31) / 32, nkg = K / 8;
    for (int t = 0; t < ntiles; ++t)
        for (int kg = 0; kg < nkg; ++kg)
            for (int lane = 0; lane < 64; ++lane) {
                const int n = t * 32 + (lane & 31), k = 8 * kg + 4 * (lane >> 5);
                float* o = out + (((size_t)t * nkg + kg) * 64 + lane) * 4;
                for (int s = 0; s < 4; ++s) o[s] = n < N ? W[(size_t)n * K + k + s] : 0.f;
            }
}

struct WeightTable {
    std::unordered_map<std::string, const gvx_weight_desc*> map;
    const float* get(const std::string& name, int64_t numel, int* rc) const {
        auto it = map.find(name);
        if (it == map.end()) { *rc = fail(GVX_ERR_MISSING_WEIGHT, "missing weight '%s'", name.c_str()); return nullptr; }
        if (it->second->numel != numel) {
            *rc = fail(GVX_ERR_SHAPE, "weight '%s' has %lld elements, expected %lld", name.c_str(), (long long)it->second->numel, (long long)numel);
            return nullptr;
        }
        return it->second->data;
    }
};

int pack_conv(const WeightTable& wt, const std::string& prefix, int cout, int cin, int k, float* w_out, float* b_out, float* u_out = nullptr) {
    int rc = GVX_OK;
    const float* w = wt.get(prefix + ".0.conv.weight", (int64_t)cout * cin * k, &rc); if (!w) return rc;
    const float* b = wt.get(prefix + ".0.conv.bias", cout, &rc); if (!b) return rc;
    const float* g = wt.get(prefix + ".1.weight", cout, &rc); if (!g) return rc;
    const float* beta = wt.get(prefix + ".1.bias", cout, &rc); if (!beta) return rc;
    const float* mu = wt.get(prefix + ".1.running_mean", cout, &rc); if (!mu) return rc;
    const float* var = wt.get(prefix + ".1.running_var", cout, &rc); if (!var) return rc;
    for (int co = 0; co < cout; ++co) {
        const double scale = (double)g[co] / std::sqrt((double)var[co] + BN_EPS);
        for (int kk = 0; kk < k; ++kk)
            for (int ci = 0; ci < cin; ++ci)
                w_out[((size_t)co * k + kk) * cin + ci] = (float)((double)w[((size_t)co * cin + ci) * k + kk] * scale);
        if (u_out)
            for (int ci = 0; ci < cin; ++ci)
                for (int s = 0; s < WINO_PTS; ++s)
                    u_out[((size_t)s * cout + co) * cin + ci] = wino_weight(w + ((size_t)co * cin + ci) * k, 1, scale, s);
        b_out[co] = (float)(((double)b[co] - (double)mu[co]) * scale + (double)beta[co]);
    }
    return GVX_OK;
}

int pack_lstm(const WeightTable& wt, const std::string& wih_name, const std::string& whh_name, const std::string& bih_name,
              const std::string& bhh_name, int Hd, int Kin, std::vector<float>* wcat, float* bias_out) {
    int rc = GVX_OK;
    const float* wih = wt.get(wih_name, (int64_t)4 * Hd * Kin, &rc); if (!wih) return rc;
    const float* whh = wt.get(whh_name, (int64_t)4 * Hd * Hd, &rc); if (!whh) return rc;
    const float* bih = wt.get(bih_name, 4 * Hd, &rc); if (!bih) return rc;
    const float* bhh = wt.get(bhh_name, 4 * Hd, &rc); if (!bhh) return rc;
    const int K = Kin + Hd;
    wcat->assign((size_t)4 * Hd * K, 0.f);
    for (int j = 0; j < Hd; ++j)
        for (int q = 0; q < 4; ++q) {
            const int src = q * Hd + j, dst = 4 * j + q;
            std::memcpy(&(*wcat)[(size_t)dst * K], wih + (size_t)src * Kin, sizeof(float) * Kin);
            std::memcpy(&(*wcat)[(size_t)dst * K + Kin], whh + (size_t)src * Hd, sizeof(float) * Hd);
            bias_out[dst] = bih[src] + bhh[src];
        }
    return GVX_OK;
}

}

extern "C" {

int gvx_model_pack_weights(gvx_model* m, const gvx_weight_desc* table, int n, void* host_blob) {
    if (!m || !table || !host_blob) return fail(GVX_ERR_INVALID_ARG, "null argument");
    WeightTable wt;
    for (int i = 0; i < n; ++i) wt.map[table[i].name] = &table[i];
    const gvx_dims& d = m->d;
    const Blob& bl = m->blob;
    float* out = reinterpret_cast<float*>(host_blob);
    std::memset(out, 0, bl.total * sizeof(float));
    const int E = d.embed_dim, H = E / 2, M = d.n_mels, P = d.prenet_dim, A = d.att_rnn_dim, D = d.dec_rnn_dim, a = d.att_dim;
    int rc = GVX_OK;
    const float* src;

    if (!(src = wt.get("embedding.weight", (int64_t)d.n_tokens * E, &rc))) return rc;
    std::memcpy(out + bl.emb, src, sizeof(float) * d.n_tokens * E);

    for (int i = 0; i < d.enc_n_conv; ++i) {
        rc = pack_conv(wt, "encoder.convolutions." + std::to_string(i), E, E, d.enc_kernel, out + bl.enc_w[i], out + bl.enc_b[i]);
        if (rc != GVX_OK) return rc;
    }
    {
        const char* sfx[2] = {"", "_reverse"};
        for (int dir = 0; dir < 2; ++dir) {
            std::vector<float> wcat;
            std::vector<float> bias(4 * H);
            rc = pack_lstm(wt, std::string("encoder.lstm.weight_ih_l0") + sfx[dir], std::string("encoder.lstm.weight_hh_l0") + sfx[dir],
                           std::string("encoder.lstm.bias_ih_l0") + sfx[dir], std::string("encoder.lstm.bias_hh_l0") + sfx[dir], H, E, &wcat, bias.data());
            if (rc != GVX_OK) return rc;
            std::vector<float> whh((size_t)4 * H * H);
            for (int r = 0; r < 4 * H; ++r) {
                std::memcpy(out + bl.enc_wih + ((size_t)dir * 4 * H + r) * E, &wcat[(size_t)r * (E + H)], sizeof(float) * E);
                std::memcpy(&whh[(size_t)r * H], &wcat[(size_t)r * (E + H) + E], sizeof(float) * H);
            }
            std::memcpy(out + bl.enc_bih + (size_t)dir * 4 * H, bias.data(), sizeof(float) * 4 * H);
            pack_frag(whh, 4 * H, H, out + bl.enc_whh_frag[dir]);
        }
    }
    {
        if (!(src = wt.get("decoder.prenet.layers.0.linear_layer.weight", (int64_t)P * M, &rc))) return rc;
        std::memcpy(out + bl.pre_w0, src, sizeof(float) * P * M);
        for (int j = 0; j < P; ++j)
            for (int k = 0; k < M; ++k) out[bl.pre_w0_t + (size_t)k * P + j] = src[(size_t)j * M + k];
        if (!(src = wt.get("decoder.prenet.layers.1.linear_layer.weight", (int64_t)P * P, &rc))) return rc;
        std::memcpy(out + bl.pre_w1, src, sizeof(float) * P * P);
        for (int j = 0; j < P; ++j)
            for (int k = 0; k < P; ++k) out[bl.pre_w1_t + (size_t)k * P + j] = src[(size_t)j * P + k];
    }
    {
        std::vector<float> wcat;
        rc = pack_lstm(wt, "decoder.attention_rnn.weight_ih", "decoder.attention_rnn.weight_hh", "decoder.attention_rnn.bias_ih",
                       "decoder.attention_rnn.bias_hh", A, P + E, &wcat, out + bl.att_bias);
        if (rc != GVX_OK) return rc;
        pack_frag(wcat, 4 * A, P + E + A, out + bl.att_frag);
        for (int n = 0; n < 4 * A; ++n) std::memcpy(out + bl.att_wpre + (size_t)n * P, &wcat[(size_t)n * (P + E + A)], sizeof(float) * P);
    }
    {
        const std::string att = "decoder.attention_layer.";
        if (!(src = wt.get(att + "query_layer.linear_layer.weight", (int64_t)a * A, &rc))) return rc;
        for (int t = 0; t < A / 8; ++t)
            for (int dd = 0; dd < a; ++dd)
                for (int jj = 0; jj < 8; ++jj) out[bl.wq_t + ((size_t)t * a + dd) * 8 + jj] = src[(size_t)dd * A + t * 8 + jj];
        if (!(src = wt.get(att + "memory_layer.linear_layer.weight", (int64_t)a * E, &rc))) return rc;
        std::memcpy(out + bl.wmem, src, sizeof(float) * a * E);
        if (!(src = wt.get(att + "v.linear_layer.weight", a, &rc))) return rc;
        std::memcpy(out + bl.v, src, sizeof(float) * a);
        const int64_t nconv = (int64_t)d.att_loc_filters * 2 * d.att_loc_kernel;
        if (!(src = wt.get(att + "location_layer.location_conv.conv.weight", nconv, &rc))) return rc;
        for (int c = 0; c < d.att_loc_filters; ++c)
            for (int ck = 0; ck < 2 * d.att_loc_kernel; ++ck) out[bl.loc_conv + (size_t)ck * 32 + c] = src[(size_t)c * 2 * d.att_loc_kernel + ck];
        if (!(src = wt.get(att + "location_layer.location_dense.linear_layer.weight", (int64_t)a * d.att_loc_filters, &rc))) return rc;
        for (int dd = 0; dd < a; ++dd)
            for (int c = 0; c < d.att_loc_filters; ++c) out[bl.loc_dense + ((size_t)(c >> 2) * a + dd) * 4 + (c & 3)] = src[(size_t)dd * d.att_loc_filters + c];
    }
    {
        std::vector<float> wcat;
        rc = pack_lstm(wt, "decoder.decoder_rnn.weight_ih", "decoder.decoder_rnn.weight_hh", "decoder.decoder_rnn.bias_ih",
                       "decoder.decoder_rnn.bias_hh", D, A + E, &wcat, out + bl.dec_bias);
        if (rc != GVX_OK) return rc;
        pack_frag(wcat, 4 * D, A + E + D, out + bl.dec_frag);
    }
    {
        const int K = D + E;
        std::vector<float> w((size_t)(M + 1) * K);
        if (!(src = wt.get("decoder.linear_projection.linear_layer.weight", (int64_t)M * K, &rc))) return rc;
        std::memcpy(w.data(), src, sizeof(float) * M * K);
        if (!(src = wt.get("decoder.gate_layer.linear_layer.weight", K, &rc))) return rc;
        std::memcpy(w.data() + (size_t)M * K, src, sizeof(float) * K);
        std::memcpy(out + bl.proj_w, w.data(), sizeof(float) * w.size());
        pack_frag(w, M + 1, K, out + bl.proj_frag);
        const int PSBp = (M + 1 + 7) & ~7;
        for (int t = 0; t < D / 8; ++t)
            for (int n = 0; n < PSBp; ++n)
                for (int jj = 0; jj < 8; ++jj)
                    out[bl.proj_hd_t + ((size_t)t * PSBp + n) * 8 + jj] = n <= M ? w[(size_t)n * K + t * 8 + jj] : 0.f;
        std::vector<float> wc((size_t)(M + 1) * E);
        for (int n = 0; n <= M; ++n) std::memcpy(&wc[(size_t)n * E], &w[(size_t)n * K + D], sizeof(float) * E);
        pack_frag(wc, M + 1, E, out + bl.proj_ctx_frag);
        for (int t = 0; t < E / 4; ++t)
            for (int n = 0; n < PSBp; ++n)
                for (int jj = 0; jj < 4; ++jj)
                    out[bl.proj_ctx_t + ((size_t)t * PSBp + n) * 4 + jj] = n <= M ? w[(size_t)n * K + D + t * 4 + jj] : 0.f;
        if (!(src = wt.get("decoder.linear_projection.linear_layer.bias", M, &rc))) return rc;
        std::memcpy(out + bl.proj_b, src, sizeof(float) * M);
        if (!(src = wt.get("decoder.gate_layer.linear_layer.bias", 1, &rc))) return rc;
        out[bl.proj_b + M] = src[0];
    }
    for (int i = 0; i < d.postnet_n_conv; ++i) {
        const int cin = i == 0 ? M : d.postnet_dim, cout = i == d.postnet_n_conv - 1 ? M : d.postnet_dim;
        rc = pack_conv(wt, "postnet.convolutions." + std::to_string(i), cout, cin, d.postnet_kernel, out + bl.post_w[i], out + bl.post_b[i],
                       postnet_layer_winograd_shape(d, i) ? out + bl.post_u[i] : nullptr);
        if (rc != GVX_OK) return rc;
    }
    return GVX_OK;
}

}

namespace {

constexpr int PACK_MAX_TENSORS = 192;
struct PackSources { const float* p[PACK_MAX_TENSORS]; };

__global__ void pack_gather_kernel(PackSources src, const int32_t* off, const uint8_t* tid, long n, float* blob) {
    for (long i = (long)blockIdx.x * blockDim.x + threadIdx.x; i < n; i += (long)gridDim.x * blockDim.x) {
        const int t = tid[i];
        if (t == 255) continue;
        blob[i] = t ? src.p[t - 1][off[i]] : 0.f;
    }
}
__global__ void pack_conv_fold_kernel(const float* w, const float* b, const float* g, const float* beta, const float* mu, const float* var,
                                      int cout, int cin, int k, float* w_out, float* b_out, float* u_out) {
    const long n = (long)cout * cin * k;
    for (long i = (long)blockIdx.x * blockDim.x + threadIdx.x; i < n; i += (long)gridDim.x * blockDim.x) {
        const int ci = (int)(i % cin), kk = (int)((i / cin) % k), co = (int)(i / ((long)cin * k));
        const double scale = (double)g[co] / sqrt((double)var[co] + BN_EPS);
        w_out[i] = (float)((double)w[((long)co * cin + ci) * k + kk] * scale);
        if (u_out && kk == 0)
            for (int s = 0; s < WINO_PTS; ++s) u_out[((long)s * cout + co) * cin + ci] = wino_weight(w + ((long)co * cin + ci) * k, 1, scale, s);
        if (ci == 0 && kk == 0) b_out[co] = (float)(((double)b[co] - (double)mu[co]) * scale + (double)beta[co]);
    }
}
__global__ void pack_lstm_bias_kernel(const float* bih, const float* bhh, int Hd, float* out) {
    const int i = blockIdx.x * blockDim.x + threadIdx.x;
    if (i < 4 * Hd) { const int j = i >> 2, q = i & 3; out[i] = bih[q * Hd + j] + bhh[q * Hd + j]; }
}

struct DevTable {
    std::unordered_map<std::string, int> idx;
    const gvx_weight_desc* t;
    const float* get(const std::string& name, int64_t numel, int* rc) const {
        auto it = idx.find(name);
        if (it == idx.end()) { *rc = fail(GVX_ERR_MISSING_WEIGHT, "missing weight '%s'", name.c_str()); return nullptr; }
        if (t[it->second].numel != numel) { *rc = fail(GVX_ERR_SHAPE, "weight '%s' has %lld elements, expected %lld", name.c_str(), (long long)t[it->second].numel, (long long)numel); return nullptr; }
        return t[it->second].data;
    }
};

int ensure_gather_map(gvx_model* m, const gvx_weight_desc* table, int n) {
    bool same = m->gather_off && (int)m->gather_names.size() == n;
    for (int i = 0; same && i < n; ++i) same = m->gather_names[i] == table[i].name && m->gather_numel[i] == table[i].numel;
    if (same) return GVX_OK;
    if (n > PACK_MAX_TENSORS || n > 254) return fail(GVX_ERR_UNSUPPORTED, "pack_weights_device: more than %d tensors", 254);
    const size_t total = m->blob.total;
    std::vector<std::vector<float>> lo(n), hi(n);
    std::vector<gvx_weight_desc> tl(n), th(n);
    for (int i = 0; i < n; ++i) {
        if (table[i].numel < 0 || table[i].numel >= (int64_t)1 << 31) return fail(GVX_ERR_UNSUPPORTED, "pack_weights_device: tensor too large");
        lo[i].resize((size_t)table[i].numel); hi[i].resize((size_t)table[i].numel);
        for (int64_t e = 0; e < table[i].numel; ++e) { lo[i][e] = (float)((e & 4095) + 1); hi[i][e] = (float)((e >> 12) * 256 + i + 1); }
        tl[i] = gvx_weight_desc{table[i].name, lo[i].data(), table[i].numel};
        th[i] = gvx_weight_desc{table[i].name, hi[i].data(), table[i].numel};
    }
    std::vector<float> bl(total), bh(total);
    int rc = gvx_model_pack_weights(m, tl.data(), n, bl.data());
    if (rc != GVX_OK) return rc;
    rc = gvx_model_pack_weights(m, th.data(), n, bh.data());
    if (rc != GVX_OK) return rc;
    std::vector<int32_t> off(total);
    std::vector<uint8_t> tid(total);
    for (size_t i = 0; i < total; ++i) {
        if (bl[i] == 0.f && bh[i] == 0.f) { off[i] = 0; tid[i] = 0; continue; }
        const long h = (long)bh[i] - 1, l = (long)bl[i] - 1;
        const int t = (int)(h % 256);
        off[i] = (int32_t)((h / 256) * 4096 + l);
        tid[i] = (uint8_t)(t + 1);
    }
    const gvx_dims& d = m->d;
    const Blob& b = m->blob;
    auto mark = [&](size_t o, size_t cnt) { std::fill(tid.begin() + o, tid.begin() + o + cnt, (uint8_t)255); };
    const int E = d.embed_dim, H = E / 2, M = d.n_mels;
    for (int i = 0; i < d.enc_n_conv; ++i) { mark(b.enc_w[i], (size_t)E * d.enc_kernel * E); mark(b.enc_b[i], E); }
    for (int i = 0; i < d.postnet_n_conv; ++i) {
        const int cin = i == 0 ? M : d.postnet_dim, cout = i == d.postnet_n_conv - 1 ? M : d.postnet_dim;
        mark(b.post_w[i], (size_t)cout * d.postnet_kernel * cin); mark(b.post_b[i], cout);
        if (postnet_layer_winograd_shape(d, i)) mark(b.post_u[i], (size_t)WINO_PTS * cout * cin);
    }
    mark(b.enc_bih, (size_t)8 * H); mark(b.att_bias, (size_t)4 * d.att_rnn_dim); mark(b.dec_bias, (size_t)4 * d.dec_rnn_dim);
    for (size_t i = 0; i < total; ++i)
        if (tid[i] && tid[i] != 255 && (tid[i] > n || off[i] < 0 || off[i] >= table[tid[i] - 1].numel))
            return fail(GVX_ERR_UNSUPPORTED, "pack_weights_device: gather map is inconsistent at blob float %zu", i);
    if (m->gather_off) { (void)hipFree(m->gather_off); m->gather_off = nullptr; }
    if (m->gather_tid) { (void)hipFree(m->gather_tid); m->gather_tid = nullptr; }
    HIP_TRY(hipMalloc(reinterpret_cast<void**>(&m->gather_off), total * sizeof(int32_t)));
    HIP_TRY(hipMalloc(reinterpret_cast<void**>(&m->gather_tid), total));
    HIP_TRY(hipMemcpy(m->gather_off, off.data(), total * sizeof(int32_t), hipMemcpyHostToDevice));
    HIP_TRY(hipMemcpy(m->gather_tid, tid.data(), total, hipMemcpyHostToDevice));
    m->gather_names.clear(); m->gather_numel.clear();
    for (int i = 0; i < n; ++i) { m->gather_names.push_back(table[i].name); m->gather_numel.push_back(table[i].numel); }
    return GVX_OK;
}

}

extern "C" {

int gvx_model_pack_weights_device(gvx_model* m, const gvx_weight_desc* table, int n, void* device_blob, void* stream) {
    if (!m || !table || !device_blob || n < 1) return fail(GVX_ERR_INVALID_ARG, "null argument");
    if (reinterpret_cast<uintptr_t>(device_blob) & 255) return fail(GVX_ERR_INVALID_ARG, "blob must be 256-byte aligned");
    int rc = ensure_gather_map(m, table, n);
    if (rc != GVX_OK) return rc;
    hipStream_t s = (hipStream_t)stream;
    float* out = reinterpret_cast<float*>(device_blob);
    PackSources src{};
    for (int i = 0; i < n; ++i) src.p[i] = table[i].data;
    const long total = (long)m->blob.total;
    hipLaunchKernelGGL(pack_gather_kernel, dim3(4096), dim3(256), 0, s, src, m->gather_off, m->gather_tid, total, out);
    DevTable dt; dt.t = table;
    for (int i = 0; i < n; ++i) dt.idx[table[i].name] = i;
    const gvx_dims& d = m->d;
    const Blob& bl = m->blob;
    const int E = d.embed_dim, H = E / 2, M = d.n_mels;
    auto conv = [&](const std::string& prefix, int cout, int cin, int k, size_t w_off, size_t b_off, const size_t* u_off = nullptr) -> int {
        int r = GVX_OK;
        const float* w = dt.get(prefix + ".0.conv.weight", (int64_t)cout * cin * k, &r); if (!w) return r;
        const float* b = dt.get(prefix + ".0.conv.bias", cout, &r); if (!b) return r;
        const float* g = dt.get(prefix + ".1.weight", cout, &r); if (!g) return r;
        const float* beta = dt.get(prefix + ".1.bias", cout, &r); if (!beta) return r;
        const float* mu = dt.get(prefix + ".1.running_mean", cout, &r); if (!mu) return r;
        const float* var = dt.get(prefix + ".1.running_var", cout, &r); if (!var) return r;
        const long cnt = (long)cout * cin * k;
        hipLaunchKernelGGL(pack_conv_fold_kernel, dim3((unsigned)((cnt + 255) / 256)), dim3(256), 0, s, w, b, g, beta, mu, var, cout, cin, k, out + w_off, out + b_off,
                           u_off ? out + *u_off : (float*)nullptr);
        return GVX_OK;
    };
    for (int i = 0; i < d.enc_n_conv; ++i)
        if ((rc = conv("encoder.convolutions." + std::to_string(i), E, E, d.enc_kernel, bl.enc_w[i], bl.enc_b[i])) != GVX_OK) return rc;
    for (int i = 0; i < d.postnet_n_conv; ++i) {
        const int cin = i == 0 ? M : d.postnet_dim, cout = i == d.postnet_n_conv - 1 ? M : d.postnet_dim;
        if ((rc = conv("postnet.convolutions." + std::to_string(i), cout, cin, d.postnet_kernel, bl.post_w[i], bl.post_b[i],
                       postnet_layer_winograd_shape(d, i) ? &bl.post_u[i] : nullptr)) != GVX_OK) return rc;
    }
    auto bias = [&](const std::string& bih_n, const std::string& bhh_n, int Hd, size_t o) -> int {
        int r = GVX_OK;
        const float* bih = dt.get(bih_n, 4 * Hd, &r); if (!bih) return r;
        const float* bhh = dt.get(bhh_n, 4 * Hd, &r); if (!bhh) return r;
        hipLaunchKernelGGL(pack_lstm_bias_kernel, dim3((4 * Hd + 255) / 256), dim3(256), 0, s, bih, bhh, Hd, out + o);
        return GVX_OK;
    };
    if ((rc = bias("encoder.lstm.bias_ih_l0", "encoder.lstm.bias_hh_l0", H, bl.enc_bih)) != GVX_OK) return rc;
    if ((rc = bias("encoder.lstm.bias_ih_l0_reverse", "encoder.lstm.bias_hh_l0_reverse", H, bl.enc_bih + (size_t)4 * H)) != GVX_OK) return rc;
    if ((rc = bias("decoder.attention_rnn.bias_ih", "decoder.attention_rnn.bias_hh", d.att_rnn_dim, bl.att_bias)) != GVX_OK) return rc;
    if ((rc = bias("decoder.decoder_rnn.bias_ih", "decoder.decoder_rnn.bias_hh", d.dec_rnn_dim, bl.dec_bias)) != GVX_OK) return rc;
    HIP_TRY(hipGetLastError());
    return GVX_OK;
}

}
```

genvox_amd/csrc/winograd_conv.hip:

```cpp
#include "gvx_kernels.h"
#include "winograd_f45.h"

namespace gvx {

namespace {

__device__ __forceinline__ float4 f4_fma(float a, const float4& x, const float4& y) {
    return make_float4(fmaf(a, x.x, y.x), fmaf(a, x.y, y.y), fmaf(a, x.z, y.z), fmaf(a, x.w, y.w));
}

__global__ void __launch_bounds__(256) winograd_input_kernel(const float* __restrict__ x, float* __restrict__ V, long mt0, long nmt, int T, int C) {
    const int tiles = (T + WINO_OUT - 1) / WINO_OUT, c4n = C >> 2;
    const long total = nmt * c4n;
    const long idx = (long)blockIdx.x * blockDim.x + threadIdx.x;
    if (idx >= total) return;
    const int c = (int)(idx % c4n) * 4;
    const long lt = idx / c4n, mt = mt0 + lt;
    const int b = (int)(mt / tiles), j = (int)(mt - (long)b * tiles);
    const int rows = T + WINO_TAPS - 1;
    const float* src = x + ((long)b * rows + 4 * j) * C + c;
    float4 d[WINO_PTS];
#pragma unroll
    for (int i = 0; i < WINO_PTS; ++i)
        d[i] = 4 * j + i < rows ? *reinterpret_cast<const float4*>(src + (long)i * C) : make_float4(0.f, 0.f, 0.f, 0.f);
    const long slice = nmt * C;
    float* dst = V + lt * C + c;
#pragma unroll
    for (int s = 0; s < WINO_PTS; ++s) {
        float4 v = make_float4(0.f, 0.f, 0.f, 0.f);
#pragma unroll
        for (int i = 0; i < WINO_PTS; ++i)
            if (wino_BT(s, i) != 0.f) v = f4_fma(wino_BT(s, i), d[i], v);
        *reinterpret_cast<float4*>(dst + s * slice) = v;
    }
}

__global__ void __launch_bounds__(256) winograd_output_kernel(const float* __restrict__ Mm, const float* __restrict__ bias, const int32_t* __restrict__ row_len,
                                                              float* __restrict__ y, long mt0, long nmt, int T, int C) {
    const int tiles = (T + WINO_OUT - 1) / WINO_OUT, c4n = C >> 2;
    const long total = nmt * c4n;
    const long idx = (long)blockIdx.x * blockDim.x + threadIdx.x;
    if (idx >= total) return;
    const int c = (int)(idx % c4n) * 4;
    const long lt = idx / c4n, mt = mt0 + lt;
    const int b = (int)(mt / tiles), j = (int)(mt - (long)b * tiles);
    const long slice = nmt * C;
    const float* src = Mm + lt * C + c;
    float4 m[WINO_PTS];
#pragma unroll
    for (int s = 0; s < WINO_PTS; ++s) m[s] = *reinterpret_cast<const float4*>(src + s * slice);
    const float4 bv = *reinterpret_cast<const float4*>(bias + c);
    const int len = row_len ? row_len[b] : T;
    constexpr int HALO = (WINO_TAPS - 1) / 2;
    const int rows = T + 2 * HALO;
    float* dst = y + ((long)b * rows + HALO) * C + c;
    const float4 zero = make_float4(0.f, 0.f, 0.f, 0.f);
#pragma unroll
    for (int i = 0; i < WINO_OUT; ++i) {
        const int t = 4 * j + i;
        float4 v = zero;
#pragma unroll
        for (int s = 0; s < WINO_PTS; ++s)
            if (wino_AT(i, s) != 0.f) v = f4_fma(wino_AT(i, s), m[s], v);
        const bool live = t < len;
        v = make_float4(live ? tanhf(v.x + bv.x) : 0.f, live ? tanhf(v.y + bv.y) : 0.f, live ? tanhf(v.z + bv.z) : 0.f, live ? tanhf(v.w + bv.w) : 0.f);
        if (t < T) *reinterpret_cast<float4*>(dst + (long)t * C) = v;
    }
    if (j == 0) {
#pragma unroll
        for (int h = 1; h <= HALO; ++h) *reinterpret_cast<float4*>(dst - (long)h * C) = zero;
    }
    if (j == tiles - 1) {
#pragma unroll
        for (int h = 0; h < HALO; ++h) *reinterpret_cast<float4*>(dst + (long)(T + h) * C) = zero;
    }
}

unsigned blocks_of(long nmt, int C) { return (unsigned)((nmt * (C >> 2) + 255) / 256); }
bool bad_shape(int B, long mt0, long nmt, int T, int C) {
    if (B < 1 || T < 1 || C < 4 || (C & 3) || mt0 < 0 || nmt < 1) return true;
    return mt0 + nmt > (long)B * ((T + WINO_OUT - 1) / WINO_OUT) || nmt * (C >> 2) > ((long)1 << 38);
}

}

hipError_t launch_winograd_input(const float* x, float* V, int B, long mt0, long nmt, int T, int C, hipStream_t s) {
    if (bad_shape(B, mt0, nmt, T, C)) return hipErrorInvalidValue;
    winograd_input_kernel<<<dim3(blocks_of(nmt, C)), dim3(256), 0, s>>>(x, V, mt0, nmt, T, C);
    return hipGetLastError();
}

hipError_t launch_winograd_output(const float* Mm, const float* bias, const int32_t* row_len, float* y, int B, long mt0, long nmt, int T, int C, hipStream_t s) {
    if (bad_shape(B, mt0, nmt, T, C)) return hipErrorInvalidValue;
    winograd_output_kernel<<<dim3(blocks_of(nmt, C)), dim3(256), 0, s>>>(Mm, bias, row_len, y, mt0, nmt, T, C);
    return hipGetLastError();
}

}
```

Baseline: 1.970 million.

## Apply Winograd convolution to encoder conv layers with ReLU output and GEMM-aligned grouping

```diff
diff --git a/genvox_amd/csrc/gemm_f32.hip b/genvox_amd/csrc/gemm_f32.hip
--- a/genvox_amd/csrc/gemm_f32.hip
+++ b/genvox_amd/csrc/gemm_f32.hip
@@ -296,6 +296,15 @@
     return pl;
 }
 
+long gemm_round_rows(const GemmParams& p) {
+    const GemmPlan pl = plan_gemm(p);
+    if (pl.err != hipSuccess || (pl.tile != 4212 && pl.tile != 2222)) return 0;
+    const long n_tiles = (long)((p.N + 127) / 128) * (p.slices > 1 ? p.slices : 1);
+    long a = 256, b = n_tiles;
+    while (b) { const long t = a % b; a = b; b = t; }
+    return 128 * (256 / a);
+}
+
 static hipError_t launch_tile(int tile, const GemmParams& p, hipStream_t s) {
     switch (tile) {
         case 4111: return launch_cfg<4, 1, 1, 1>(p, s);
diff --git a/genvox_amd/csrc/gvx_api.hip b/genvox_amd/csrc/gvx_api.hip
--- a/genvox_amd/csrc/gvx_api.hip
+++ b/genvox_amd/csrc/gvx_api.hip
@@ -52,6 +52,20 @@
     const size_t tile = (size_t)2 * WINO_PTS * m->d.postnet_dim, all = (size_t)B * ((T + WINO_OUT - 1) / WINO_OUT) * tile;
     const size_t budget = WINOGRAD_GROUP_BYTES / sizeof(float) / tile * tile;
     return all <= budget ? all : budget > tile ? budget : tile;
+}
+
+long winograd_group_tiles(long total, long fit, int C) {
+    if (fit >= total) return total;
+    const long groups = (total + fit - 1) / fit, per = (total + groups - 1) / groups;
+    GemmParams g{};
+    g.M = (int)per; g.N = C; g.K = C; g.slices = WINO_PTS;
+    const long unit = gemm_round_rows(g);
+    if (unit <= 0) return per;
+    auto whole = [&](long rows) { g.M = (int)rows; return rows > 0 && rows <= fit && rows % unit == 0 && gemm_round_rows(g) == unit; };
+    const long down = per / unit * unit, up = (per + unit - 1) / unit * unit, most = fit / unit * unit;
+    if (whole(down) && total - (groups - 1) * down <= fit) return down;
+    if (whole(up)) return up;
+    return whole(most) ? most : per;
 }
 
 WsPlan make_ws_plan(const gvx_model* m, int B, int L, int T, int mode) {
@@ -168,7 +182,7 @@
     m->ar_resident = flag("GVX_AR_RESIDENT", false);
     m->ar_split_h = flag("GVX_AR_SPLIT_H", true);
     m->enc_persistent = flag("GVX_ENC_PERSISTENT", true);
-    m->enc_fork_after = number("GVX_ENC_FORK_AFTER", 1);
+    m->enc_fork_after = number("GVX_ENC_FORK_AFTER", 2);
     m->train_resident = flag("GVX_TRAIN_RESIDENT", true);
     m->train_resident_loop = flag("GVX_TRAIN_RESIDENT_LOOP", true);
     m->tf_rows64 = flag("GVX_TF_ROWS64", false);
@@ -268,9 +282,41 @@
     return GVX_OK;
 }
 
+int winograd_layer(const gvx_model* m, const char* who, const float* cur, float* nxt, int B, int T, int C, size_t u_off, size_t b_off,
+                   const int32_t* row_len, int act, float* wino, size_t wino_floats, hipStream_t s) {
+    const long total = (long)B * ((T + WINO_OUT - 1) / WINO_OUT);
+    const size_t tile = (size_t)2 * WINO_PTS * C, budget = WINOGRAD_GROUP_BYTES / sizeof(float);
+    long fit = (long)((wino_floats < budget ? wino_floats : budget) / tile);
+    if (fit < 1) return fail(GVX_ERR_WORKSPACE, "%s: %zu floats of scratch do not hold one Winograd tile (%zu)", who, wino_floats, tile);
+    if (m->wino_group > 0 && m->wino_group < fit) fit = m->wino_group;
+    const long per_group = winograd_group_tiles(total, fit, C);
+    for (long mt0 = 0, Mt; mt0 < total; mt0 += Mt) {
+        Mt = total - mt0 <= fit ? total - mt0 : per_group;
+        float* V = wino;
+        float* Mm = wino + (size_t)WINO_PTS * Mt * C;
+        HIP_TRY(launch_winograd_input(cur, V, B, mt0, Mt, T, C, s));
+        GemmParams g{};
+        g.A = V; g.amap = RowMap{(int)Mt, 0, (long)C};
+        g.W = m->dev_blob + u_off; g.ldw = C;
+        g.C = Mm; g.cmap = RowMap{(int)Mt, 0, (long)C};
+        g.bias = nullptr; g.M = (int)Mt; g.N = C; g.K = C; g.act = ACT_NONE;
+        g.slices = WINO_PTS; g.a_slice = Mt * C; g.w_slice = (long)C * C; g.c_slice = Mt * C;
+        HIP_TRY(launch_gemm(g, s));
+        HIP_TRY(launch_winograd_output(Mm, m->dev_blob + b_off, row_len, nxt, B, mt0, Mt, T, C, act, s));
+    }
+    return GVX_OK;
+}
+
+struct WinoScratch { size_t off, floats; };
+WinoScratch encoder_wino_scratch(const WsPlan& wp, bool alone) {
+    if (alone) return {wp.xg, (wp.total - wp.xg) / sizeof(float)};
+    const size_t front = wp.frames - wp.xg, back = wp.pre_gate - wp.h_a;
+    return front >= back ? WinoScratch{wp.xg, front / sizeof(float)} : WinoScratch{wp.h_a, back / sizeof(float)};
+}
+
 int encoder_impl(gvx_model* m, const int64_t* tokens, const int32_t* lengths, int B, int L, float* memory_out, void* ws,
-                 const WsPlan& wp, hipStream_t s, const float* conv_out = nullptr, float* c_seq_out = nullptr, float* xg_out = nullptr,
-                 hipEvent_t dense_done = nullptr) {
+                 const WsPlan& wp, const WinoScratch& wsc, hipStream_t s, const float* conv_out = nullptr, float* c_seq_out = nullptr,
+                 float* xg_out = nullptr, hipEvent_t dense_done = nullptr) {
     const gvx_dims& d = m->d;
     const int E = d.embed_dim, H = E / 2, pe = (d.enc_kernel - 1) / 2;
     float* xa = ws_ptr<float>(ws, wp.xa);
@@ -287,7 +333,10 @@
         HIP_TRY(launch_embed(tokens, m->dev_blob + m->blob.emb, d.n_tokens, xa, xb, B, L, E, pe, flags + FLAG_TOKEN, s));
         for (int i = 0; i < d.enc_n_conv; ++i) {
             if (dense_done && i == m->enc_fork_after) { HIP_TRY(hipEventRecord(dense_done, s)); dense_done = nullptr; }
-            int rc = conv_layer(m, cur, nxt, B, L, E, E, d.enc_kernel, m->blob.enc_w[i], m->blob.enc_b[i], ACT_RELU, pe, s);
+            const bool wino = encoder_layer_winograd_shape(d, i) && conv_uses_winograd(m, E, E, d.enc_kernel);
+            int rc = wino ? winograd_layer(m, "encoder", cur, nxt, B, L, E, m->blob.enc_u[i], m->blob.enc_b[i], nullptr, ACT_RELU,
+                                           ws_ptr<float>(ws, wsc.off), wsc.floats, s)
+                          : conv_layer(m, cur, nxt, B, L, E, E, d.enc_kernel, m->blob.enc_w[i], m->blob.enc_b[i], ACT_RELU, pe, s);
             if (rc != GVX_OK) return rc;
             float* t = cur; cur = nxt; nxt = t;
         }
@@ -372,28 +421,8 @@
         const int cin = i == 0 ? M : d.postnet_dim, cout = i == n - 1 ? M : d.postnet_dim;
         const bool last = i == n - 1;
         if (postnet_layer_winograd_shape(d, i) && conv_uses_winograd(m, cin, cout, d.postnet_kernel)) {
-            const int C = cin;
-            const long total = (long)B * ((T + WINO_OUT - 1) / WINO_OUT);
-            const size_t tile = (size_t)2 * WINO_PTS * C, budget = WINOGRAD_GROUP_BYTES / sizeof(float);
-            long fit = (long)((wino_floats < budget ? wino_floats : budget) / tile);
-            if (fit < 1) return fail(GVX_ERR_WORKSPACE, "Postnet: %zu floats of scratch do not hold one Winograd tile (%zu)", wino_floats, tile);
-            if (m->wino_group > 0 && m->wino_group < fit) fit = m->wino_group;
-            if (fit > total) fit = total;
-            const long groups = (total + fit - 1) / fit, per_group = (total + groups - 1) / groups;
-            for (long mt0 = 0; mt0 < total; mt0 += per_group) {
-                const long Mt = total - mt0 < per_group ? total - mt0 : per_group;
-                float* V = wino;
-                float* Mm = wino + (size_t)WINO_PTS * Mt * C;
-                HIP_TRY(launch_winograd_input(cur, V, B, mt0, Mt, T, C, s));
-                GemmParams g{};
-                g.A = V; g.amap = RowMap{(int)Mt, 0, (long)C};
-                g.W = m->dev_blob + m->blob.post_u[i]; g.ldw = C;
-                g.C = Mm; g.cmap = RowMap{(int)Mt, 0, (long)C};
-                g.bias = nullptr; g.M = (int)Mt; g.N = C; g.K = C; g.act = ACT_NONE;
-                g.slices = WINO_PTS; g.a_slice = Mt * C; g.w_slice = (long)C * C; g.c_slice = Mt * C;
-                HIP_TRY(launch_gemm(g, s));
-                HIP_TRY(launch_winograd_output(Mm, m->dev_blob + m->blob.post_b[i], mel_lengths, nxt, B, mt0, Mt, T, C, s));
-            }
+            const int rc = winograd_layer(m, "Postnet", cur, nxt, B, T, cin, m->blob.post_u[i], m->blob.post_b[i], mel_lengths, ACT_TANH, wino, wino_floats, s);
+            if (rc != GVX_OK) return rc;
             float* t = cur; cur = nxt; nxt = t;
             continue;
         }
@@ -509,6 +538,11 @@
     if (!m || tiles < 0) return fail(GVX_ERR_INVALID_ARG, "bad argument");
     m->wino_group = tiles;
     return GVX_OK;
+}
+
+long gvx_debug_winograd_group_tiles(long total, long fit, int channels) {
+    if (total < 1 || fit < 1 || channels < 4 || total > INT_MAX) return -1;
+    return winograd_group_tiles(total, fit, channels);
 }
 
 int gvx_debug_winograd_constants(double* at, double* g, double* bt) {
@@ -555,7 +589,8 @@
     int rc = check_common(m, B, L, 1, ws, ws_bytes, WS_AUTOREGRESSIVE);
     if (rc != GVX_OK) return rc;
     if (!tokens || !memory_out) return fail(GVX_ERR_INVALID_ARG, "null argument");
-    return encoder_impl(m, tokens, lengths, B, L, memory_out, ws, make_ws_plan(m, B, L, 1, WS_AUTOREGRESSIVE), (hipStream_t)stream);
+    const WsPlan wp = make_ws_plan(m, B, L, 1, WS_AUTOREGRESSIVE);
+    return encoder_impl(m, tokens, lengths, B, L, memory_out, ws, wp, encoder_wino_scratch(wp, true), (hipStream_t)stream);
 }
 
 int gvx_decoder_teacher_forced(gvx_model* m, const float* memory, const int32_t* lengths, int B, int L, const float* mel_in, int T,
@@ -578,8 +613,9 @@
     if (rc != GVX_OK) return rc;
     if (!conv_out || !memory_out) return fail(GVX_ERR_INVALID_ARG, "null argument");
     if (cell_states_out) HIP_TRY(zero_async(cell_states_out, (size_t)B * L * m->d.embed_dim * sizeof(float), (hipStream_t)stream));
-    return encoder_impl(m, nullptr, lengths, B, L, memory_out, ws, make_ws_plan(m, B, L, 1, WS_AUTOREGRESSIVE), (hipStream_t)stream, conv_out,
-                        cell_states_out, input_preact_out);
+    const WsPlan wp = make_ws_plan(m, B, L, 1, WS_AUTOREGRESSIVE);
+    return encoder_impl(m, nullptr, lengths, B, L, memory_out, ws, wp, encoder_wino_scratch(wp, true), (hipStream_t)stream, conv_out, cell_states_out,
+                        input_preact_out);
 }
 
 int gvx_decoder_teacher_forced_train(gvx_model* m, const float* memory, const int32_t* lengths, int B, int L, const float* mel_in, int T,
@@ -627,6 +663,7 @@
         case 1: HIP_TRY(hipMemcpyAsync(dst, ws_ptr<float>(ws, wp.pre1), rows * d.prenet_dim * sizeof(float), hipMemcpyDeviceToDevice, s)); break;
         case 2: return gvx_train_unblock(ws_ptr<float>(ws, wp.prenet), dst, T + 1, B, d.prenet_dim, stream);
         case 3: HIP_TRY(hipMemcpyAsync(dst, ws_ptr<float>(ws, wp.pm), (size_t)B * L * d.att_dim * sizeof(float), hipMemcpyDeviceToDevice, s)); break;
+        case 4: HIP_TRY(hipMemcpyAsync(dst, ws_ptr<float>(ws, wp.memory), (size_t)B * L * d.embed_dim * sizeof(float), hipMemcpyDeviceToDevice, s)); break;
         default: return fail(GVX_ERR_INVALID_ARG, "gvx_train_export: unknown buffer %d", what);
     }
     return GVX_OK;
@@ -676,7 +713,7 @@
         if (rc != GVX_OK) return rc;
         HIP_TRY(hipEventRecord(m->pa_fork, s));
         HIP_TRY(hipStreamWaitEvent(m->pa_stream, m->pa_fork, 0));
-        rc = encoder_impl(m, tokens, token_lengths, B, L, memory, ws, wp, m->pa_stream, nullptr, nullptr, nullptr, m->enc_mid);
+        rc = encoder_impl(m, tokens, token_lengths, B, L, memory, ws, wp, encoder_wino_scratch(wp, false), m->pa_stream, nullptr, nullptr, nullptr, m->enc_mid);
         if (rc != GVX_OK) return rc;
         rc = decoder_init_states(m, memory, B, L, decoder_buffers(ws, wp), m->pa_stream);
         if (rc != GVX_OK) return rc;
@@ -686,7 +723,7 @@
         if (rc != GVX_OK) return rc;
         HIP_TRY(hipStreamWaitEvent(s, m->pa_join, 0));
     } else {
-        rc = encoder_impl(m, tokens, token_lengths, B, L, memory, ws, wp, s);
+        rc = encoder_impl(m, tokens, token_lengths, B, L, memory, ws, wp, encoder_wino_scratch(wp, false), s);
         if (rc != GVX_OK) return rc;
     }
     if (timed) HIP_TRY(hipEventRecord(m->ev[1], s));
diff --git a/genvox_amd/csrc/gvx_internal.h b/genvox_amd/csrc/gvx_internal.h
--- a/genvox_amd/csrc/gvx_internal.h
+++ b/genvox_amd/csrc/gvx_internal.h
@@ -36,11 +36,15 @@
     size_t proj_w, proj_b, proj_frag, proj_hd_t, proj_ctx_frag, proj_ctx_t;
     size_t post_w[MAX_CONV], post_b[MAX_CONV];
     size_t post_u[MAX_CONV];
+    size_t enc_u[MAX_CONV];
     size_t total;
 };
 inline bool winograd_shape_ok(int cin, int cout, int k) { return k == WINO_TAPS && cin == cout && cin % 32 == 0; }
 inline bool postnet_layer_winograd_shape(const gvx_dims& d, int i) {
     return i > 0 && i < d.postnet_n_conv - 1 && winograd_shape_ok(d.postnet_dim, d.postnet_dim, d.postnet_kernel);
+}
+inline bool encoder_layer_winograd_shape(const gvx_dims& d, int i) {
+    return i >= 0 && i < d.enc_n_conv && winograd_shape_ok(d.embed_dim, d.embed_dim, d.enc_kernel);
 }
 Blob make_blob_layout(const gvx_dims& d);
 
@@ -76,7 +80,7 @@
     bool attn_prefetch = true;
     int winograd = 1;
     int wino_group = 0;
-    int enc_fork_after = 1;
+    int enc_fork_after = 2;
     int pa_depth = 4;
     unsigned side_pool = 1;
     unsigned spin_limit = 0;
@@ -169,6 +173,7 @@
 constexpr int WINOGRAD_MIN_CHANNELS = 256;
 constexpr size_t WINOGRAD_GROUP_BYTES = (size_t)128 << 20;
 bool conv_uses_winograd(const gvx_model* m, int cin, int cout, int k);
+long winograd_group_tiles(long total, long fit, int C);
 size_t winograd_scratch_floats(const gvx_model* m, int B, int T);
 
 constexpr int FLAG_TOKEN = 0;
diff --git a/genvox_amd/csrc/gvx_kernels.h b/genvox_amd/csrc/gvx_kernels.h
--- a/genvox_amd/csrc/gvx_kernels.h
+++ b/genvox_amd/csrc/gvx_kernels.h
@@ -44,6 +44,7 @@
 hipError_t launch_gemm(const GemmParams& p, hipStream_t s);
 struct GemmPlan { hipError_t err; int tile; int rows_big; };
 GemmPlan plan_gemm(const GemmParams& p);
+long gemm_round_rows(const GemmParams& p);
 void set_splitk(GemmParams& p, int splitk);
 hipError_t launch_gemm_splitk(const GemmParams& p, int splitk, float* scratch, hipStream_t s);
 
@@ -274,7 +275,7 @@
                                              const int32_t* lens, hipStream_t s);
 hipError_t launch_zero_halo(float* buf, int B, int T, int halo, int C, hipStream_t s);
 hipError_t launch_winograd_input(const float* x, float* V, int B, long mt0, long nmt, int T, int C, hipStream_t s);
-hipError_t launch_winograd_output(const float* M, const float* bias, const int32_t* row_len, float* y, int B, long mt0, long nmt, int T, int C, hipStream_t s);
+hipError_t launch_winograd_output(const float* M, const float* bias, const int32_t* row_len, float* y, int B, long mt0, long nmt, int T, int C, int act, hipStream_t s);
 hipError_t launch_mask_padding(float* mel, float* mel_post, float* gate, const int32_t* mel_lengths, int B, int M, int T,
                                hipStream_t s);
 hipError_t launch_zero_many(void* const* ptrs, const size_t* bytes, int n_arrays, hipStream_t s);
diff --git a/genvox_amd/csrc/gvx_pack.hip b/genvox_amd/csrc/gvx_pack.hip
--- a/genvox_amd/csrc/gvx_pack.hip
+++ b/genvox_amd/csrc/gvx_pack.hip
@@ -36,6 +36,8 @@
     }
     for (int i = 0; i < d.postnet_n_conv; ++i)
         if (postnet_layer_winograd_shape(d, i)) b.post_u[i] = take((size_t)WINO_PTS * d.postnet_dim * d.postnet_dim);
+    for (int i = 0; i < d.enc_n_conv; ++i)
+        if (encoder_layer_winograd_shape(d, i)) b.enc_u[i] = take((size_t)WINO_PTS * E * E);
     b.total = off;
     return b;
 }
@@ -129,7 +131,8 @@
     std::memcpy(out + bl.emb, src, sizeof(float) * d.n_tokens * E);
 
     for (int i = 0; i < d.enc_n_conv; ++i) {
-        rc = pack_conv(wt, "encoder.convolutions." + std::to_string(i), E, E, d.enc_kernel, out + bl.enc_w[i], out + bl.enc_b[i]);
+        rc = pack_conv(wt, "encoder.convolutions." + std::to_string(i), E, E, d.enc_kernel, out + bl.enc_w[i], out + bl.enc_b[i],
+                       encoder_layer_winograd_shape(d, i) ? out + bl.enc_u[i] : nullptr);
         if (rc != GVX_OK) return rc;
     }
     {
@@ -302,7 +305,10 @@
     const Blob& b = m->blob;
     auto mark = [&](size_t o, size_t cnt) { std::fill(tid.begin() + o, tid.begin() + o + cnt, (uint8_t)255); };
     const int E = d.embed_dim, H = E / 2, M = d.n_mels;
-    for (int i = 0; i < d.enc_n_conv; ++i) { mark(b.enc_w[i], (size_t)E * d.enc_kernel * E); mark(b.enc_b[i], E); }
+    for (int i = 0; i < d.enc_n_conv; ++i) {
+        mark(b.enc_w[i], (size_t)E * d.enc_kernel * E); mark(b.enc_b[i], E);
+        if (encoder_layer_winograd_shape(d, i)) mark(b.enc_u[i], (size_t)WINO_PTS * E * E);
+    }
     for (int i = 0; i < d.postnet_n_conv; ++i) {
         const int cin = i == 0 ? M : d.postnet_dim, cout = i == d.postnet_n_conv - 1 ? M : d.postnet_dim;
         mark(b.post_w[i], (size_t)cout * d.postnet_kernel * cin); mark(b.post_b[i], cout);
@@ -357,7 +363,8 @@
         return GVX_OK;
     };
     for (int i = 0; i < d.enc_n_conv; ++i)
-        if ((rc = conv("encoder.convolutions." + std::to_string(i), E, E, d.enc_kernel, bl.enc_w[i], bl.enc_b[i])) != GVX_OK) return rc;
+        if ((rc = conv("encoder.convolutions." + std::to_string(i), E, E, d.enc_kernel, bl.enc_w[i], bl.enc_b[i],
+                       encoder_layer_winograd_shape(d, i) ? &bl.enc_u[i] : nullptr)) != GVX_OK) return rc;
     for (int i = 0; i < d.postnet_n_conv; ++i) {
         const int cin = i == 0 ? M : d.postnet_dim, cout = i == d.postnet_n_conv - 1 ? M : d.postnet_dim;
         if ((rc = conv("postnet.convolutions." + std::to_string(i), cout, cin, d.postnet_kernel, bl.post_w[i], bl.post_b[i],
diff --git a/genvox_amd/csrc/winograd_conv.hip b/genvox_amd/csrc/winograd_conv.hip
--- a/genvox_amd/csrc/winograd_conv.hip
+++ b/genvox_amd/csrc/winograd_conv.hip
@@ -35,6 +35,7 @@
     }
 }
 
+template <int ACT>
 __global__ void __launch_bounds__(256) winograd_output_kernel(const float* __restrict__ Mm, const float* __restrict__ bias, const int32_t* __restrict__ row_len,
                                                               float* __restrict__ y, long mt0, long nmt, int T, int C) {
     const int tiles = (T + WINO_OUT - 1) / WINO_OUT, c4n = C >> 2;
@@ -50,7 +51,7 @@
 #pragma unroll
     for (int s = 0; s < WINO_PTS; ++s) m[s] = *reinterpret_cast<const float4*>(src + s * slice);
     const float4 bv = *reinterpret_cast<const float4*>(bias + c);
-    const int len = row_len ? row_len[b] : T;
+    [[maybe_unused]] const int len = row_len ? row_len[b] : T;
     constexpr int HALO = (WINO_TAPS - 1) / 2;
     const int rows = T + 2 * HALO;
     float* dst = y + ((long)b * rows + HALO) * C + c;
@@ -62,8 +63,12 @@
 #pragma unroll
         for (int s = 0; s < WINO_PTS; ++s)
             if (wino_AT(i, s) != 0.f) v = f4_fma(wino_AT(i, s), m[s], v);
-        const bool live = t < len;
-        v = make_float4(live ? tanhf(v.x + bv.x) : 0.f, live ? tanhf(v.y + bv.y) : 0.f, live ? tanhf(v.z + bv.z) : 0.f, live ? tanhf(v.w + bv.w) : 0.f);
+        if constexpr (ACT == ACT_TANH) {
+            const bool live = t < len;
+            v = make_float4(live ? tanhf(v.x + bv.x) : 0.f, live ? tanhf(v.y + bv.y) : 0.f, live ? tanhf(v.z + bv.z) : 0.f, live ? tanhf(v.w + bv.w) : 0.f);
+        } else {
+            v = make_float4(fmaxf(v.x + bv.x, 0.f), fmaxf(v.y + bv.y, 0.f), fmaxf(v.z + bv.z, 0.f), fmaxf(v.w + bv.w, 0.f));
+        }
         if (t < T) *reinterpret_cast<float4*>(dst + (long)t * C) = v;
     }
     if (j == 0) {
@@ -90,9 +95,10 @@
     return hipGetLastError();
 }
 
-hipError_t launch_winograd_output(const float* Mm, const float* bias, const int32_t* row_len, float* y, int B, long mt0, long nmt, int T, int C, hipStream_t s) {
-    if (bad_shape(B, mt0, nmt, T, C)) return hipErrorInvalidValue;
-    winograd_output_kernel<<<dim3(blocks_of(nmt, C)), dim3(256), 0, s>>>(Mm, bias, row_len, y, mt0, nmt, T, C);
+hipError_t launch_winograd_output(const float* Mm, const float* bias, const int32_t* row_len, float* y, int B, long mt0, long nmt, int T, int C, int act, hipStream_t s) {
+    if (bad_shape(B, mt0, nmt, T, C) || (act != ACT_TANH && (act != ACT_RELU || row_len))) return hipErrorInvalidValue;
+    if (act == ACT_TANH) winograd_output_kernel<ACT_TANH><<<dim3(blocks_of(nmt, C)), dim3(256), 0, s>>>(Mm, bias, row_len, y, mt0, nmt, T, C);
+    else winograd_output_kernel<ACT_RELU><<<dim3(blocks_of(nmt, C)), dim3(256), 0, s>>>(Mm, bias, nullptr, y, mt0, nmt, T, C);
     return hipGetLastError();
 }
 
```

Measured after the change: 2.005 million (median of 6 runs). +1.8%, better.
